# jujuC31/NeutFEM

Hardware: AMD Instinct MI355X
Metric: outer power-iters/sec (IAEA-3D RT0-P0 k-eigenvalue solve) (higher is better)
Workload: dtype f64; 1 GPU; IAEA-3D resampled 256x256x256 RT0-P0 2g, full Schur path, CG tol 0.0001, Chebyshev; cells=16777216, groups=2, parallelism=1 process(es) x 1 z-slab(s) each; RCCL: interface planes + scalar all-reduces

## Files before the change

### neutfem_amd/csrc/neutfem_hip.hip

```cpp
#include "../../include/neutfem_hip.h"
#include "nf_kernels.h"
#include "nf_assembly.h"
#include "nf_line_groups.h"
#include "nf_options.h"
#include "nf_small_eig.h"

#include <dlfcn.h>
#include <unistd.h>

#include <algorithm>
#include <chrono>
#include <climits>
#include <cmath>
#include <cstdarg>
#include <cstdint>
#include <cstdio>
#include <cstdlib>
#include <cstring>
#include <map>
#include <mutex>
#include <string>
#include <type_traits>
#include <utility>
#include <vector>

using namespace nf;

static thread_local std::string g_err;
static int fail(int code, const char *fmt, ...)
{
    char buf[512]; va_list ap; va_start(ap, fmt); vsnprintf(buf, sizeof buf, fmt, ap); va_end(ap);
    g_err = buf; return code;
}
#define HIPCHK(x) do { hipError_t e_ = (x); if (e_ != hipSuccess) return fail(NF_ERR_HIP, "%s failed: %s (%s:%d)", #x, hipGetErrorString(e_), __FILE__, __LINE__); } while (0)
#define NFCHK(x) do { int r_ = (x); if (r_ != NF_OK) return r_; } while (0)

static_assert(NF_OPT_RED_GRID == 1024, "nf_options.h: defaults and cap of the reduction-shaped grids follow RED_GRID");
static const int RED_GRID = 1024;
static const int MAX_LOCAL_SLABS = 16;

struct ProfSlot {
    std::vector<float> samples;
    void stats(long *count, double *ms, long *skipped) const
    {
        *count = 0; *ms = 0.0; *skipped = 0;
        if (samples.empty()) return;
        std::vector<float> v(samples); std::nth_element(v.begin(), v.begin() + v.size() / 2, v.end());
        const double thr = 0.25 * v[v.size() / 2];
        for (float x : samples) { if (x < thr) ++*skipped; else { ++*count; *ms += x; } }
    }
};

typedef struct ncclComm *ncclComm_t;
typedef struct { char internal[128]; } ncclUniqueId;
struct Rccl {
    void *lib = nullptr;
    int (*GetUniqueId)(ncclUniqueId *) = nullptr;
    int (*CommInitRank)(ncclComm_t *, int, ncclUniqueId, int) = nullptr;
// ... 2 lines not shown
    int (*Send)(const void *, size_t, int, int, ncclComm_t, hipStream_t) = nullptr;
    int (*Recv)(void *, size_t, int, int, ncclComm_t, hipStream_t) = nullptr;
    int (*GroupStart)() = nullptr;
    int (*GroupEnd)() = nullptr;
    const char *(*GetErrorString)(int) = nullptr;
    int (*CommAbort)(ncclComm_t) = nullptr;
    int (*CommCount)(const ncclComm_t, int *) = nullptr;
    char path[512] = { 0 };
};
static Rccl g_rccl;
static bool trace_comm() { static int on = -1; if (on < 0) { const char *e = getenv("NEUTFEM_TRACE_COMM"); on = e && atoi(e) ? 1 : 0; } return on == 1; }
#define TRACE_COMM(...) do { if (trace_comm()) { fprintf(stderr, "[comm] " __VA_ARGS__); fputc('\n', stderr); } } while (0)
static const int NCCL_DOUBLE = 8, NCCL_SUM = 0, NCCL_MAX = 2;
#define NCCLCHK(x) do { int r_ = (x); if (r_ != 0) return fail(NF_ERR_HIP, "%s failed: %s", #x, g_rccl.GetErrorString ? g_rccl.GetErrorString(r_) : "rccl error"); } while (0)

static int rccl_load()
{
    if (g_rccl.lib) return NF_OK;
    const char *env = getenv("NEUTFEM_RCCL_LIB");
    const char *names[] = { env ? env : "/opt/rocm/lib/librccl.so.1", "/opt/rocm/lib/librccl.so.1", "librccl.so.1", "librccl.so" };
    for (const char *n : names) { g_rccl.lib = dlopen(n, RTLD_NOW | RTLD_LOCAL); if (g_rccl.lib) break; }
    if (!g_rccl.lib) return fail(NF_ERR_HIP, "cannot load librccl.so: %s", dlerror());
#define SYM(field, name) do { *(void **)(&g_rccl.field) = dlsym(g_rccl.lib, name); if (!g_rccl.field) return fail(NF_ERR_HIP, "librccl.so lacks %s", name); } while (0)
    SYM(GetUniqueId, "ncclGetUniqueId"); SYM(CommInitRank, "ncclCommInitRank"); SYM(CommDestroy, "ncclCommDestroy");
    SYM(AllReduce, "ncclAllReduce"); SYM(Send, "ncclSend"); SYM(Recv, "ncclRecv"); SYM(GroupStart, "ncclGroupStart");
    SYM(GroupEnd, "ncclGroupEnd"); SYM(GetErrorString, "ncclGetErrorString");
#undef SYM
    *(void **)(&g_rccl.CommAbort) = dlsym(g_rccl.lib, "ncclCommAbort");
    *(void **)(&g_rccl.CommCount) = dlsym(g_rccl.lib, "ncclCommCount");
    Dl_info di;
    if (dladdr((void *)g_rccl.AllReduce, &di) && di.dli_fname) snprintf(g_rccl.path, sizeof g_rccl.path, "%s", di.dli_fname);
    return NF_OK;
}

struct nf_solver;
struct Transient;
struct nf_team {
    NfOptions opt;
    std::vector<nf_solver *> slabs;
    int device = 0;
    hipStream_t stream = nullptr;
    hipStream_t comm_stream = nullptr;
    hipStream_t y_stream = nullptr; hipEvent_t ev_fork = nullptr, ev_join = nullptr;
    hipEvent_t ev_z1 = nullptr, ev_xchg = nullptr;
    int nproc = 1, rank = 0;
    ncclComm_t comm = nullptr;
    ncclComm_t comm_x = nullptr;
    int last_cg_reductions = 0; long team_max_cells = 0;
    int last_cg_form = 0;
    int last_endpoint_w = 0;
    bool rccl_reduce = false;
    double *d_partials = nullptr; long partial_stride = 0, slab_cap = 0;
    CgScalars *d_cg = nullptr;
    double *d_out = nullptr;
    double *d_red = nullptr;
    double *d_errsrc = nullptr;
    double *d_vec = nullptr; long vec_stride = 0;
    int vec_cnt_pq = 0, vec_cnt_rr = 0; bool vec_ok = false; int last_vec_reduce = 0;
    bool dead = false;
    bool poisoned = false; int poison_rc = 0; char poison_msg[256] = { 0 };
    int xchg_in_apply = 0;
    long cg_iter_total = 0;
    int inject_rank = -1; long inject_iter = -1;
    int inject_outer = -1; char inject_where = 0;
    double comm_timeout_s = 120.0;
    nf_progress_fn progress_fn = nullptr; void *progress_user = nullptr;
    volatile long outers_done = 0;
    bool linked_ready = false;
    int sep_sweeps = 0;
    std::vector<int> last_its;
    int last_outer = 0, coarse_outer = 0; long last_cg_total = 0;
    std::vector<double> hist_k, hist_dk, hist_dphi; std::vector<int> hist_cg;
    int has_valid_keff = 0; double last_keff = 1.0;
    HostPub *h_pub = nullptr, *d_pub = nullptr; unsigned long long pub_seq = 0;
    bool profile = false; long prof_tick = 0;
    std::map<std::string, ProfSlot> prof;
    struct Ev { hipEvent_t a, b; int slot; };
    std::vector<Ev> ev_pending; std::vector<std::pair<hipEvent_t, hipEvent_t>> ev_free;
    OuterState *d_ost = nullptr; double *d_hist = nullptr; int hist_cap = 0;
    int ncu = 256;
    size_t lds_limit = 160 * 1024;
    int last_xcd = 0; long xcd_solves = 0, xcd_refused = 0;
    XcdState *d_xcd = nullptr; double *d_xpart = nullptr;
    int last_resident_serial = 0;
    int *d_hist_cg = nullptr; int hist_cg_cap = 0; ResidentOut *d_rout = nullptr;
    int last_path = 0;
    int last_direct = 0;
    long standin_unconverged = 0;
    std::vector<nf_solver *> cc; int cc_f[3] = {0, 0, 0};
};

struct nf_solver {
    int device = 0;
    nf_team *team = nullptr;
    int slab_index = 0;
    int if_lo = 0, if_hi = 0;
    int dim = 1, nx = 1, ny = 1, nz = 1, ng = 1, k = 0, m = 0;
    int n1 = 1, nloc = 1, nb = 0;
    long N = 0, nphi = 0, nJ = 0, nJx = 0, nJy = 0, nJz = 0;
    std::vector<double> xb, yb, zb, hx, hy, hz;
    double *d_hx = nullptr, *d_hy = nullptr, *d_hz = nullptr, *d_xb = nullptr, *d_yb = nullptr, *d_zb = nullptr;
    int bc_set[8] = {0}, bc_type[8] = {0};
    double *d_D = nullptr, *d_SigR = nullptr, *d_NSF = nullptr, *d_Chi = nullptr;
    std::vector<double *> d_SigS;
    bool xs_uploaded = false, built = false, diag_valid = false;
    unsigned char *d_void = nullptr; std::vector<unsigned char> void_host; double void_gamma = 0.0; long void_cells = 0;
    double *d_Cd = nullptr, *d_Mf = nullptr, *d_Mchi = nullptr;
    double *d_phi_adj = nullptr;
    double *d_modes[2] = {nullptr, nullptr}; int modes_n[2] = {0, 0}, modes_cap[2] = {0, 0};
    int has_valid_adjoint = 0; double last_keff_adj = 1.0;
    double *d_gamma = nullptr, *d_gpt_w = nullptr, *d_gpt_sc = nullptr; bool gpt_valid = false;
    std::vector<double *> d_Ms;
    const double **d_Ms_tab = nullptr;
    double *d_L[3] = {nullptr, nullptr, nullptr}, *d_DR[3] = {nullptr, nullptr, nullptr}, *d_D0[3] = {nullptr, nullptr, nullptr};
    long nlines[3] = {0, 0, 0};
    bool ld_tried = false, ld_use[3] = {false, false, false}; int ld_rejected = 0, ld_pitch[3] = {0, 0, 0};
    int *d_lid[3] = {nullptr, nullptr, nullptr}; double *d_ltab[3] = {nullptr, nullptr, nullptr};
    std::vector<long> ld_off[3]; std::vector<int> ld_rows[3]; size_t ld_bytes = 0;
    double *d_Sinv = nullptr;
    double *d_Sdense = nullptr; bool dense_valid = false;
    double *d_alo = nullptr, *d_ahi = nullptr, *d_hlo = nullptr, *d_hhi = nullptr, *d_gfl = nullptr;
    double *d_sinv_lo = nullptr, *d_sinv_hi = nullptr;
    double *d_clo = nullptr, *d_chi = nullptr, *d_rlo = nullptr, *d_rhi = nullptr, *d_ulo = nullptr, *d_uhi = nullptr;
    double *d_ctlo = nullptr, *d_cthi = nullptr, *d_elo = nullptr, *d_ehi = nullptr, *d_relo = nullptr, *d_rehi = nullptr;
    double *d_Wlo = nullptr, *d_Whi = nullptr; bool w_valid = false;
    double *d_phi = nullptr, *d_raw = nullptr;
    double *d_p0 = nullptr, *d_p1 = nullptr;
    double *d_tf = nullptr, *d_rhs = nullptr, *d_r = nullptr, *d_p = nullptr, *d_q = nullptr;
    double *d_p2 = nullptr, *d_qy = nullptr, *d_qz = nullptr;
    bool raw_valid = false, raw_is_diag = false;
    double *d_qsrc = nullptr;
    double src_total = 0.0; bool src_any = false;
    Transient *tr = nullptr; long build_gen = 0;
    long tr_rebuilds = 0;
    int opt_tr_rebalance = 1;
    double *d_Jz = nullptr; bool jz_valid = false;
    double *d_Jzb = nullptr;
    bool cmfd_init = false, cmfd_iface = false; double cmfd_relax = 1.0;
    double *d_Dt[3] = {nullptr, nullptr, nullptr}, *d_Dh[3] = {nullptr, nullptr, nullptr}; long nfc[3] = {0, 0, 0};
    double *d_cm = nullptr, *d_cmJ = nullptr; CmfdScalars *d_cmsc = nullptr;
    int cmfd_last_its = 0;
};

const char *nf_last_error(void) { return g_err.c_str(); }

static void coarse_cache_drop(nf_team *T)
{
    if (!T || T->cc.empty()) return;
    std::string keep = g_err;
    std::vector<nf_solver *> cc; cc.swap(T->cc);
    for (int i = (int)cc.size() - 1; i >= 0; --i) if (cc[i]) nf_destroy(cc[i]);
    g_err = keep;
}

int nf_device_count(void)
{
    int n = 0;
    if (hipGetDeviceCount(&n) != hipSuccess) { (void)hipGetLastError(); return 0; }
    return n;
}

template <class T> static int dalloc(T **p, size_t n)
{
    if (*p) { (void)hipFree(*p); *p = nullptr; }
    HIPCHK(hipMalloc((void **)p, std::max<size_t>(n, 1) * sizeof(T)));
    return NF_OK;
}
template <class T> static void dfree(T *&p) { if (p) { (void)hipFree(p); p = nullptr; } }
template <class T> struct DevTmp { T *p = nullptr; ~DevTmp() { if (p) (void)hipFree(p); } DevTmp() = default; DevTmp(const DevTmp &) = delete; DevTmp &operator=(const DevTmp &) = delete; };

static void line_dict_drop(nf_solver *S)
{
    if (S->team && S->team->stream && (S->d_lid[0] || S->d_lid[1] || S->d_lid[2])) (void)hipStreamSynchronize(S->team->stream);
    for (int d = 0; d < 3; ++d) { dfree(S->d_lid[d]); dfree(S->d_ltab[d]); S->ld_use[d] = false; S->ld_pitch[d] = 0; S->ld_off[d].clear(); S->ld_rows[d].clear(); }
    S->ld_tried = false; S->ld_rejected = 0; S->ld_bytes = 0;
}

static void modes_drop(nf_solver *S);
static void gpt_drop(nf_solver *S);
static void transient_drop(nf_solver *S);
static bool team_is_single(const nf_team *T);
// ... 37 lines not shown
    long g = (n + block - 1) / block; if (g < 1) g = 1; if (g > cap) g = cap; return (int)g;
}

static int n_modes(const nf_solver *S) { int n = 1; for (int t = 1; t < S->dim; ++t) n *= S->n1; return n; }
static int moment_index(const nf_solver *S, int d, int mode, int i, double *Ta)
{
    const int n1 = S->n1;
    int idx[3] = {0, 0, 0}; double ta = 1.0; int q = mode;
    for (int t = 0; t < S->dim; ++t) {
        if (t == d) { idx[t] = i; continue; }
        idx[t] = q % n1; q /= n1;
        ta *= 2.0 / (2.0 * idx[t] + 1.0);
    }
    if (Ta) *Ta = ta;
    return idx[0] + n1 * idx[1] + n1 * n1 * idx[2];
}
static ModeArgs mode_args(const nf_solver *S, int g, int d, int mode, const double *xb, double *yb)
{
    ModeArgs ma; memset(&ma, 0, sizeof ma);
    double Ta = 1.0;
    for (int i = 0; i <= S->nb; ++i) {
        const int p = moment_index(S, d, mode, i, &Ta);
        ma.x[i] = xb + (long)p * S->N; ma.y[i] = yb + (long)p * S->N; ma.Cd[i] = S->d_Cd + (long)g * S->nphi + (long)p * S->N;
    }
    ma.Ta = Ta; ma.dir = d; ma.D = S->d_D + (long)g * S->N;
    ma.eL[0] = 5.0 / 8.0; ma.eR[0] = 5.0 / 8.0; ma.Gc[0] = -4.0 / 3.0; ma.iM[0] = 15.0 / 16.0;
    ma.eL[1] = -7.0 / 8.0; ma.eR[1] = 7.0 / 8.0; ma.Gc[1] = -4.0 / 5.0; ma.iM[1] = 105.0 / 16.0;
    return ma;
}
static ModeTab mode_tab(const nf_solver *S, int d)
{
    ModeTab mt; memset(&mt, 0, sizeof mt);
    mt.n = n_modes(S);
    for (int m = 0; m < mt.n; ++m)
        for (int i = 0; i <= S->nb; ++i) {
            double Ta = 1.0;
            const int p = moment_index(S, d, m, i, &Ta), p0 = moment_index(S, d, 0, i, nullptr);
            mt.Ta[m] = Ta; mt.doff[m][i] = (long)(p - p0) * S->N;
        }
    return mt;
}

static long slab_partial_need(const nf_solver *S)
{
    return (std::max<long>(RED_GRID, S->nlines[0] + (long)((S->nx + 7) / 8) * ((long)S->ny + S->nz)) + 16) * n_modes(S);
}
static int team_alloc(nf_team *T)
{
    long cap = 0;
    for (auto *S : T->slabs) cap = std::max(cap, slab_partial_need(S));
    T->slab_cap = cap; T->partial_stride = cap * (long)T->slabs.size();
    NFCHK(dalloc(&T->d_partials, (size_t)T->partial_stride * 4));
    if (!T->d_cg) NFCHK(dalloc(&T->d_cg, 1));
    if (!T->d_out) NFCHK(dalloc(&T->d_out, 8));
    if (!T->d_red) NFCHK(dalloc(&T->d_red, 8));
    if (!T->d_errsrc) { NFCHK(dalloc(&T->d_errsrc, 1)); HIPCHK(hipMemset(T->d_errsrc, 0, sizeof(double))); }
    if (const char *e = getenv("NEUTFEM_INJECT_FAIL")) {
        int r = -1, ml = 0; long it = -1; char w = 0; int on = -1;
        if (sscanf(e, "%d:%c%d", &r, &w, &on) >= 2 && (w == 'o' || w == 'e' || w == 'a')) { T->inject_rank = r; T->inject_where = w; T->inject_outer = on; }
        else {
            const int nf = sscanf(e, "%d:%ld:%d", &r, &it, &ml);
            if (nf >= 2 && (nf < 3 || T->slabs.empty() || T->slabs[0]->nloc >= ml)) { T->inject_rank = r; T->inject_iter = it; }
        }
    }
    if (const char *e = getenv("NEUTFEM_COMM_TIMEOUT_S")) { const double v = atof(e); if (v > 0) T->comm_timeout_s = v; }
    T->last_its.assign(64, 0);
    return NF_OK;
}
static void team_free(nf_team *T)
{
    if (!T) return;
    (void)hipSetDevice(T->device);
    if (T->dead) {
        delete T;
        return;
    }
    if (T->stream) (void)hipStreamSynchronize(T->stream);
    for (auto &e : T->ev_pending) { (void)hipEventDestroy(e.a); (void)hipEventDestroy(e.b); }
    for (auto &e : T->ev_free) { (void)hipEventDestroy(e.first); (void)hipEventDestroy(e.second); }
    if (T->comm_x && g_rccl.CommDestroy) g_rccl.CommDestroy(T->comm_x);
    if (T->comm && g_rccl.CommDestroy) g_rccl.CommDestroy(T->comm);
    if (T->d_xcd) (void)hipFree(T->d_xcd);
    dfree(T->d_xpart);
    dfree(T->d_partials); dfree(T->d_cg); dfree(T->d_out); dfree(T->d_red); dfree(T->d_errsrc); dfree(T->d_vec); dfree(T->d_ost); dfree(T->d_hist); dfree(T->d_hist_cg); dfree(T->d_rout);
    if (T->h_pub) (void)hipHostFree(T->h_pub);
    if (T->comm_stream) { (void)hipStreamSynchronize(T->comm_stream); (void)hipStreamDestroy(T->comm_stream); }
    if (T->y_stream) { (void)hipStreamSynchronize(T->y_stream); (void)hipStreamDestroy(T->y_stream); }
    if (T->ev_fork) (void)hipEventDestroy(T->ev_fork);
    if (T->ev_join) (void)hipEventDestroy(T->ev_join);
    if (T->ev_z1) (void)hipEventDestroy(T->ev_z1);
    if (T->ev_xchg) (void)hipEventDestroy(T->ev_xchg);
    if (T->stream) (void)hipStreamDestroy(T->stream);
    delete T;
}
static PartSegs segs_for(const nf_team *T, const std::vector<int> &counts)
{
    PartSegs ps; ps.n = (int)T->slabs.size();
    for (int i = 0; i < ps.n; ++i) { ps.off[i] = (int)(i * T->slab_cap); ps.cnt[i] = counts[i]; }
    return ps;
}

static int create_impl(int rt_order, int p_order, int ng, int nxb, const double *xb, int nyb, const double *yb, int nzb,
                       const double *zb, int if_lo, int if_hi, int device, nf_handle *out)
{
    if (!out || !xb || nxb < 2 || ng < 1 || ng > 64) return fail(NF_ERR_ARG, "nf_create: bad arguments");
    int k = std::min(rt_order, 2), m = std::min(p_order, 2);
    if (k < m) m = k;
    int ndev = nf_device_count();
    if (ndev <= 0) return fail(NF_ERR_NO_DEVICE, "nf_create: no HIP device visible (the gfx950 path has no CPU fallback)");
    if (device < 0 || device >= ndev) return fail(NF_ERR_ARG, "nf_create: device %d out of range (%d devices)", device, ndev);
    HIPCHK(hipSetDevice(device));
    nf_solver *S = new nf_solver();
    S->device = device; S->k = k; S->m = m; S->ng = ng; S->if_lo = if_lo; S->if_hi = if_hi;
    S->xb.assign(xb, xb + nxb);
    if (nyb > 1) S->yb.assign(yb, yb + nyb); else S->yb.assign(1, nyb == 1 && yb ? yb[0] : 0.0);
    if (nzb > 1) S->zb.assign(zb, zb + nzb); else S->zb.assign(1, nzb == 1 && zb ? zb[0] : 0.0);
    S->nx = nxb - 1; S->ny = nyb > 1 ? nyb - 1 : 1; S->nz = nzb > 1 ? nzb - 1 : 1;
    S->dim = S->nz > 1 ? 3 : (S->ny > 1 ? 2 : 1);
    if ((if_lo || if_hi) && (S->dim != 3 || S->nz < 3)) { delete S; return fail(NF_ERR_ARG, "a slab needs a 3D mesh with at least 3 z-planes"); }
    if (S->dim == 3 && (nyb < 2 || !yb)) { delete S; return fail(NF_ERR_ARG, "nf_create: a 3D mesh needs at least 2 y breaks (got %d)", nyb); }
    S->N = (long)S->nx * S->ny * S->nz;
    S->n1 = m + 1; S->nloc = 1; for (int t = 0; t < S->dim; ++t) S->nloc *= S->n1;
    S->nphi = S->N * S->nloc; S->nb = std::min(k, m);
    S->hx.resize(S->nx); S->hy.assign(S->ny, 1.0); S->hz.assign(S->nz, 1.0);
    for (int i = 0; i < S->nx; ++i) S->hx[i] = xb[i + 1] - xb[i];
    if (S->dim >= 2) for (int i = 0; i < S->ny; ++i) S->hy[i] = yb[i + 1] - yb[i];
    if (S->dim == 3) for (int i = 0; i < S->nz; ++i) S->hz[i] = zb[i + 1] - zb[i];
    for (auto *h : { &S->hx, &S->hy, &S->hz })
        for (double v : *h)
            if (!(v > 0.0) || !std::isfinite(v)) { delete S; return fail(NF_ERR_ARG, "nf_create: mesh breaks must be finite and strictly increasing (cell width %g)", v); }
    {
        int nf = 1, ni = k; for (int t = 1; t < S->dim; ++t) { nf *= k + 1; ni *= k + 1; }
        S->nJx = (long)(S->nx + 1) * S->ny * S->nz * nf;
        S->nJy = S->dim >= 2 ? (long)S->nx * (S->ny + 1) * S->nz * nf : 0;
        S->nJz = S->dim == 3 ? (long)S->nx * S->ny * (S->nz + 1) * nf : 0;
        S->nJ = S->nJx + S->nJy + S->nJz + S->N * S->dim * ni;
    }
// ... 46 lines not shown
    if (rc == NF_OK) rc = dalloc(&S->d_q, S->nphi);
    if (rc == NF_OK && (if_lo || if_hi)) {
        const size_t nl = (size_t)S->nlines[2] * n_modes(S);
        double **arrs[] = { &S->d_clo, &S->d_chi, &S->d_rlo, &S->d_rhi, &S->d_ulo, &S->d_uhi, &S->d_ctlo, &S->d_cthi, &S->d_elo, &S->d_ehi, &S->d_relo, &S->d_rehi };
        for (auto a : arrs) if (rc == NF_OK) { rc = dalloc(a, nl); if (rc == NF_OK) (void)hipMemset(*a, 0, nl * sizeof(double)); }
    }
    if (rc == NF_OK) rc = team_alloc(T);
    if (rc != NF_OK) { nf_destroy(S); *out = nullptr; return rc; }
    S->d_SigS.assign((size_t)ng * ng, nullptr); S->d_Ms.assign((size_t)ng * ng, nullptr);
    return nf_reset_flux(S);
}

int nf_create(int rt_order, int p_order, int ng, int nxb, const double *xb, int nyb, const double *yb, int nzb,
              const double *zb, int device, nf_handle *out)
{
    return create_impl(rt_order, p_order, ng, nxb, xb, nyb, yb, nzb, zb, 0, 0, device, out);
}
int nf_create_slab(int rt_order, int p_order, int ng, int nxb, const double *xb, int nyb, const double *yb, int nzb,
                   const double *zb_slab, int interface_below, int interface_above, int device, nf_handle *out)
{
    return create_impl(rt_order, p_order, ng, nxb, xb, nyb, yb, nzb, zb_slab, interface_below ? 1 : 0, interface_above ? 1 : 0, device, out);
}

int nf_destroy(nf_handle S)
{
    if (!S) return NF_OK;
    (void)hipSetDevice(S->device);
    nf_team *T = S->team;
    if (T && T->dead) {
        std::vector<nf_solver *> cc; cc.swap(T->cc);
        for (auto *c : cc) if (c) nf_destroy(c);
        T->slabs.erase(std::remove(T->slabs.begin(), T->slabs.end(), S), T->slabs.end());
        if (T->slabs.empty()) team_free(T);
        delete S;
        return NF_OK;
    }
    coarse_cache_drop(T);
    transient_drop(S);
    if (T && T->stream) (void)hipStreamSynchronize(T->stream);
    for (int d = 0; d < 3; ++d) { dfree(S->d_Dt[d]); dfree(S->d_Dh[d]); }
    dfree(S->d_cm); dfree(S->d_cmJ); dfree(S->d_cmsc);
    dfree(S->d_hx); dfree(S->d_hy); dfree(S->d_hz); dfree(S->d_xb); dfree(S->d_yb); dfree(S->d_zb);
    dfree(S->d_D); dfree(S->d_SigR); dfree(S->d_NSF); dfree(S->d_Chi); dfree(S->d_void);
    for (auto &p : S->d_SigS) dfree(p);
    for (auto &p : S->d_Ms) dfree(p);
    dfree(S->d_Ms_tab);
    dfree(S->d_Cd); dfree(S->d_Mf); dfree(S->d_Mchi); dfree(S->d_phi_adj); dfree(S->d_Sinv); dfree(S->d_Sdense);
    for (int d = 0; d < 3; ++d) { dfree(S->d_L[d]); dfree(S->d_DR[d]); dfree(S->d_D0[d]); dfree(S->d_lid[d]); dfree(S->d_ltab[d]); }
    dfree(S->d_alo); dfree(S->d_ahi); dfree(S->d_hlo); dfree(S->d_hhi); dfree(S->d_gfl); dfree(S->d_sinv_lo); dfree(S->d_sinv_hi);
    dfree(S->d_clo); dfree(S->d_chi); dfree(S->d_rlo); dfree(S->d_rhi); dfree(S->d_ulo); dfree(S->d_uhi);
    dfree(S->d_Wlo); dfree(S->d_Whi);
    dfree(S->d_Jz); dfree(S->d_Jzb); dfree(S->d_ctlo); dfree(S->d_cthi); dfree(S->d_elo); dfree(S->d_ehi); dfree(S->d_relo); dfree(S->d_rehi);
    dfree(S->d_phi); dfree(S->d_raw); dfree(S->d_p0); dfree(S->d_p1);
    dfree(S->d_tf); dfree(S->d_rhs); dfree(S->d_r); dfree(S->d_p); dfree(S->d_q); dfree(S->d_p2); dfree(S->d_qy); dfree(S->d_qz);
    dfree(S->d_qsrc); dfree(S->d_modes[0]); dfree(S->d_modes[1]);
    dfree(S->d_gamma); dfree(S->d_gpt_w); dfree(S->d_gpt_sc);
    if (T) {
        T->slabs.erase(std::remove(T->slabs.begin(), T->slabs.end(), S), T->slabs.end());
        for (size_t i = 0; i < T->slabs.size(); ++i) T->slabs[i]->slab_index = (int)i;
        if (T->slabs.empty()) team_free(T);
    }
    delete S;
    return NF_OK;
}

int nf_link_slabs(nf_handle *handles, int n)
{
    if (!handles || n < 1 || n > MAX_LOCAL_SLABS) return fail(NF_ERR_ARG, "nf_link_slabs: 1..%d slabs", MAX_LOCAL_SLABS);
    nf_solver *S0 = handles[0];
    if (!S0) return fail(NF_ERR_ARG, "nf_link_slabs: null handle");
    HIPCHK(hipSetDevice(S0->device));
    for (int i = 0; i < n; ++i) {
        nf_solver *S = handles[i];
        if (!S || S->team->slabs.size() != 1) return fail(NF_ERR_STATE, "nf_link_slabs: handle %d is null or already linked", i);
        if (S->device != S0->device || S->nx != S0->nx || S->ny != S0->ny || S->ng != S0->ng)
            return fail(NF_ERR_ARG, "nf_link_slabs: slab %d does not match slab 0 (device, nx, ny, groups)", i);
        if (i > 0 && (!S->if_lo || !handles[i - 1]->if_hi)) return fail(NF_ERR_ARG, "nf_link_slabs: slabs %d/%d lack the shared interface flag", i - 1, i);
    }
    nf_team *T = S0->team;
    for (int i = 0; i < n; ++i) coarse_cache_drop(handles[i]->team);
    for (int i = 1; i < n; ++i) {
        nf_solver *S = handles[i];
        team_free(S->team);
        S->team = T; S->slab_index = i; T->slabs.push_back(S);
    }
    T->linked_ready = false;
    return team_alloc(T);
}

int nf_comm_unique_id(void *id128)
{
    if (!id128) return fail(NF_ERR_ARG, "nf_comm_unique_id: null buffer");
    NFCHK(rccl_load());
    ncclUniqueId id; NCCLCHK(g_rccl.GetUniqueId(&id));
    memcpy(id128, &id, sizeof id);
    return NF_OK;
}
int nf_comm_init(nf_handle S, const void *id128, int nranks, int rank)
{
    if (!S || !id128 || nranks < 1 || rank < 0 || rank >= nranks) return fail(NF_ERR_ARG, "nf_comm_init: bad arguments");
    nf_team *T = S->team;
    const bool force = getenv("NEUTFEM_FORCE_RCCL") != nullptr;
    if (nranks == 1 && !force) { T->nproc = 1; T->rank = 0; return NF_OK; }
    NFCHK(rccl_load());
    HIPCHK(hipSetDevice(T->device));
    ncclUniqueId id; memcpy(&id, id128, sizeof id);
    NCCLCHK(g_rccl.CommInitRank(&T->comm, nranks, id, rank));
// ... 311 lines not shown
}
static void prof_collect(nf_team *T)
{
    for (auto &e : T->ev_pending) {
        float ms = 0.f;
        if (hipEventSynchronize(e.b) == hipSuccess && hipEventElapsedTime(&ms, e.a, e.b) == hipSuccess) T->prof[SLOT_NAMES[e.slot]].samples.push_back(ms);
        T->ev_free.push_back({e.a, e.b});
    }
    T->ev_pending.clear();
}

static int exchange_planes(nf_team *T, int which, int g, hipStream_t st)
{
    const int ns = (int)T->slabs.size();
    ++T->xchg_in_apply;
    auto send_lo = [&](nf_solver *S) { return which == 0 ? S->d_clo : which == 2 ? S->d_elo : S->d_hlo + (size_t)g * S->nlines[2]; };
    auto send_hi = [&](nf_solver *S) { return which == 0 ? S->d_chi : which == 2 ? S->d_ehi : S->d_hhi + (size_t)g * S->nlines[2]; };
    auto recv_lo = [&](nf_solver *S) { return which == 2 ? S->d_relo : S->d_rlo; };
    auto recv_hi = [&](nf_solver *S) { return which == 2 ? S->d_rehi : S->d_rhi; };
    for (int i = 0; i + 1 < ns; ++i) {
        nf_solver *A = T->slabs[i], *B = T->slabs[i + 1];
        const size_t bytes = (size_t)A->nlines[2] * (which == 1 ? 1 : n_modes(A)) * sizeof(double);
        HIPCHK(hipMemcpyAsync(recv_lo(B), send_hi(A), bytes, hipMemcpyDeviceToDevice, st));
        HIPCHK(hipMemcpyAsync(recv_hi(A), send_lo(B), bytes, hipMemcpyDeviceToDevice, st));
    }
    nf_solver *bot = T->slabs.front(), *top = T->slabs.back();
    if (T->nproc > 1 && (bot->if_lo || top->if_hi)) {
        const size_t cnt = (size_t)bot->nlines[2] * (which == 1 ? 1 : n_modes(bot));
        TRACE_COMM("rank %d exchange which=%d count=%zu lo=%d hi=%d poisoned=%d", T->rank, which, cnt, bot->if_lo, top->if_hi, (int)T->poisoned);
        ncclComm_t cx = T->comm_x ? T->comm_x : T->comm;
        NCCLCHK(g_rccl.GroupStart());
        if (bot->if_lo) {
            NCCLCHK(g_rccl.Send(send_lo(bot), cnt, NCCL_DOUBLE, T->rank - 1, cx, st));
            NCCLCHK(g_rccl.Recv(recv_lo(bot), cnt, NCCL_DOUBLE, T->rank - 1, cx, st));
        }
        if (top->if_hi) {
            NCCLCHK(g_rccl.Send(send_hi(top), cnt, NCCL_DOUBLE, T->rank + 1, cx, st));
            NCCLCHK(g_rccl.Recv(recv_hi(top), cnt, NCCL_DOUBLE, T->rank + 1, cx, st));
        }
        NCCLCHK(g_rccl.GroupEnd());
    } else if (bot->if_lo || top->if_hi) {
        return fail(NF_ERR_STATE, "slab %s has an interface but no neighbour: link the slabs (nf_link_slabs) or init the communicator (nf_comm_init)",
                    bot->if_lo ? "bottom" : "top");
    }
    return NF_OK;
}

struct ApplyCg {
    const CgScalars *cg = nullptr;
    bool fused = false; const std::vector<double *> *xsol = nullptr;
    CgLean lean = {};
    CgLean lean_z1 = {};
    Cg1 cg1 = {};
};
struct PassCg {
    const CgScalars *cg = nullptr; CgFuse fuse = {}; CgLean lean = {}, lean_z1 = {}; Cg1 cg1 = {};
    bool zw_dot = false;
    hipStream_t stream = nullptr;
    bool noacc = false; const double *yadd = nullptr;
};
static PassCg pass_cg(const ApplyCg &A, const nf_solver *S, int i) { return { A.cg, A.fused ? CgFuse{ S->d_p, S->d_r, (*A.xsol)[i] } : CgFuse{}, A.lean, A.lean_z1, A.cg1 }; }
struct SegPlan { int rc = NF_OK, SEG = 0, NSEG = 0, TX = 0, nparts = 0; dim3 grid, block; size_t lds = 0; };
static SegPlan seg_plan(const nf_solver *S, int d, int zmode);
static int launch_s(const nf_solver *S, int d, int g, const ModeArgs &ma, const Geom &G, int last, double *partials, const PassCg &P, int *nparts, int zmode);
static int line_dict_prepare(nf_team *T);
static int team_prepare(nf_team *T)
{
    NFCHK(line_dict_prepare(T));
    if (T->linked_ready) return NF_OK;
    if (T->opt.xchg_comm && T->nproc > 1 && T->comm && !T->comm_x) {
        ncclUniqueId id2; memset(&id2, 0, sizeof id2);
        double v[128]; for (double &x : v) x = 0.0;
        if (T->rank == 0) { NCCLCHK(g_rccl.GetUniqueId(&id2)); for (int i = 0; i < 128; ++i) v[i] = (double)(unsigned char)id2.internal[i]; }
        DevTmp<double> d; NFCHK(dalloc(&d.p, 128));
        HIPCHK(hipMemcpyAsync(d.p, v, sizeof v, hipMemcpyHostToDevice, T->stream));
        NCCLCHK(g_rccl.AllReduce(d.p, d.p, 128, NCCL_DOUBLE, NCCL_SUM, T->comm, T->stream));
        HIPCHK(hipMemcpyAsync(v, d.p, sizeof v, hipMemcpyDeviceToHost, T->stream));
        NFCHK(team_stream_wait(T, T->stream));
        for (int i = 0; i < 128; ++i) id2.internal[i] = (char)(unsigned char)v[i];
        NCCLCHK(g_rccl.CommInitRank(&T->comm_x, T->nproc, id2, T->rank));
        TRACE_COMM("rank %d: second communicator for the plane exchange", T->rank);
    }
    bool any = false;
    for (auto *S : T->slabs) { if (!S->built) return fail(NF_ERR_STATE, "every slab must be built (nf_build) before solving"); any |= S->if_lo || S->if_hi; }
    if (any) {
        const int ng = T->slabs[0]->ng;
        for (int g = 0; g < ng; ++g) {
            NFCHK(exchange_planes(T, 1, g, T->stream));
            for (auto *S : T->slabs) {
                const long nl = S->nlines[2];
                const unsigned gr = (unsigned)((nl + 255) / 256);
                if (S->if_lo) hipLaunchKernelGGL(k_sred_inv, dim3(gr), dim3(256), 0, T->stream, S->d_hlo + g * nl, S->d_rlo, S->d_sinv_lo + g * nl, nl, 0);
                if (S->if_hi) hipLaunchKernelGGL(k_sred_inv, dim3(gr), dim3(256), 0, T->stream, S->d_hhi + g * nl, S->d_rhi, S->d_sinv_hi + g * nl, nl, 1);
            }
            NFCHK(team_stream_wait(T, T->stream));
        }
        double worst = 0.0; int worst_nz = 0;
        for (auto *S : T->slabs) {
            if (!(S->if_lo && S->if_hi)) continue;
            const size_t nl = (size_t)S->nlines[2] * ng;
            std::vector<double> gfl(nl), slo(nl), shi(nl);
            HIPCHK(hipMemcpy(gfl.data(), S->d_gfl, nl * sizeof(double), hipMemcpyDeviceToHost));
            HIPCHK(hipMemcpy(slo.data(), S->d_sinv_lo, nl * sizeof(double), hipMemcpyDeviceToHost));
            HIPCHK(hipMemcpy(shi.data(), S->d_sinv_hi, nl * sizeof(double), hipMemcpyDeviceToHost));
            for (size_t i = 0; i < nl; ++i) {
                const double w = std::fabs(gfl[i]) * std::sqrt(std::fabs(slo[i] * shi[i]));
                if (w > worst) { worst = w; worst_nz = S->nz; }
            }
        }
        if (T->rccl_reduce && T->nproc > 1) {
            HIPCHK(hipMemcpyAsync(T->d_red, &worst, sizeof(double), hipMemcpyHostToDevice, T->stream));
            NCCLCHK(g_rccl.AllReduce(T->d_red, T->d_red, 1, NCCL_DOUBLE, NCCL_MAX, T->comm, T->stream));
            HIPCHK(hipMemcpyAsync(&worst, T->d_red, sizeof(double), hipMemcpyDeviceToHost, T->stream));
            NFCHK(team_stream_wait(T, T->stream));
// ... 13 lines not shown
    T->vec_ok = false;
    T->team_max_cells = 0; for (auto *X : T->slabs) T->team_max_cells = std::max(T->team_max_cells, X->N);
    if (T->rccl_reduce && T->nproc > 1) {
        nf_solver *S = T->slabs[0];
        const bool eligible = T->slabs.size() == 1 && S->nloc == 1 && S->dim == 3 && (S->if_lo || S->if_hi);
        int np = 0;
        if (eligible) {
            const SegPlan sp = seg_plan(S, 2, 2);
            np = sp.rc == NF_OK ? sp.nparts : 0;
        }
        const int nr = eligible ? grid_for(S->nphi) : 0;
        double v[5] = { (double)np, -(double)np, (double)nr, -(double)nr, (double)T->team_max_cells };
        HIPCHK(hipMemcpyAsync(T->d_red, v, sizeof v, hipMemcpyHostToDevice, T->stream));
        NCCLCHK(g_rccl.AllReduce(T->d_red, T->d_red, 5, NCCL_DOUBLE, NCCL_MAX, T->comm, T->stream));
        HIPCHK(hipMemcpyAsync(v, T->d_red, sizeof v, hipMemcpyDeviceToHost, T->stream));
        NFCHK(team_stream_wait(T, T->stream));
        T->team_max_cells = (long)v[4];
        T->vec_cnt_pq = np; T->vec_cnt_rr = nr;
        T->vec_stride = T->slab_cap + 2;
        T->vec_ok = eligible && v[0] == -v[1] && v[2] == -v[3] && np > 0 && np < T->slab_cap && nr > 0 && nr < T->slab_cap;
        if (T->vec_ok && !T->d_vec) { NFCHK(dalloc(&T->d_vec, (size_t)T->vec_stride * 2)); HIPCHK(hipMemset(T->d_vec, 0, (size_t)T->vec_stride * 2 * sizeof(double))); }
    }
    for (auto *S : T->slabs) S->w_valid = false;
    if (T->opt.endpoint_weights && T->opt.cg_single_reduce != 0 && (T->opt.cg_single_reduce > 0 || T->team_max_cells <= T->opt.cg_single_reduce_max_cells))
        for (auto *S : T->slabs) {
            if (!(S->if_lo || S->if_hi) || S->nb != 0 || S->dim != 3 || S->nloc != 1) continue;
            const size_t NG = (size_t)S->N * S->ng; const long nxy = S->nlines[2];
            if (!S->d_Wlo) { NFCHK(dalloc(&S->d_Wlo, NG)); NFCHK(dalloc(&S->d_Whi, NG)); }
            HIPCHK(hipMemsetAsync(S->d_Wlo, 0, NG * sizeof(double), T->stream)); HIPCHK(hipMemsetAsync(S->d_Whi, 0, NG * sizeof(double), T->stream));
            HIPCHK(hipMemsetAsync(S->d_p, 0, (size_t)S->N * sizeof(double), T->stream));
            const Geom G = make_geom(S);
            const unsigned gf = (unsigned)grid_for(nxy);
            for (int g = 0; g < S->ng; ++g)
                for (int k = 0; k < S->nz; ++k) {
                    double *plane = S->d_p + (size_t)k * nxy;
                    hipLaunchKernelGGL(k_fill_const, dim3(gf), dim3(256), 0, T->stream, plane, nxy, 1.0);
                    NFCHK(launch_s(S, 2, g, mode_args(S, g, 2, 0, S->d_p, S->d_q), G, 0, nullptr, PassCg(), nullptr, 1));
                    if (S->if_lo) HIPCHK(hipMemcpyAsync(S->d_Wlo + (size_t)g * S->N + (size_t)k * nxy, S->d_clo, (size_t)nxy * sizeof(double), hipMemcpyDeviceToDevice, T->stream));
                    if (S->if_hi) HIPCHK(hipMemcpyAsync(S->d_Whi + (size_t)g * S->N + (size_t)k * nxy, S->d_chi, (size_t)nxy * sizeof(double), hipMemcpyDeviceToDevice, T->stream));
                    hipLaunchKernelGGL(k_fill_const, dim3(gf), dim3(256), 0, T->stream, plane, nxy, 0.0);
                }
            HIPCHK(hipStreamSynchronize(T->stream));
            HIPCHK(hipGetLastError());
            S->w_valid = true;
        }
    T->linked_ready = true;
    return NF_OK;
}

static int team_finalize(nf_team *T, int op, const std::vector<int> &counts, int nq, double *out, double tol, int maxit, bool want_flag = false)
{
    PartSegs ps = segs_for(T, counts);
    if (!T->rccl_reduce) {
        hipLaunchKernelGGL(k_finalize, dim3(1), dim3(256), 0, T->stream, op, T->d_partials, ps, T->partial_stride, nq, T->d_cg, out, tol, maxit, 0, T->d_red, (const double *)nullptr);
    } else {
        hipLaunchKernelGGL(k_finalize, dim3(1), dim3(256), 0, T->stream, op, T->d_partials, ps, T->partial_stride, nq, T->d_cg, out, tol, maxit, 1, T->d_red, (const double *)T->d_errsrc);
        TRACE_COMM("rank %d allreduce finalize op=%d count=%d poisoned=%d", T->rank, op, nq + 1, (int)T->poisoned);
        NCCLCHK(g_rccl.AllReduce(T->d_red, T->d_red, (size_t)nq + 1, NCCL_DOUBLE, NCCL_SUM, T->comm, T->stream));
        hipLaunchKernelGGL(k_cg_logic, dim3(1), dim3(1), 0, T->stream, op, T->d_red, nq, T->d_cg, out, tol, maxit, want_flag ? 2 : 1);
    }
    return NF_OK;
}

static bool team_poison(nf_team *T, int code, bool vec_slots = false)
{
    if (code == NF_OK) return false;
    if (T->nproc <= 1) return true;
    if (!T->poisoned) {
        T->poisoned = true; T->poison_rc = code; snprintf(T->poison_msg, sizeof T->poison_msg, "%s", nf_last_error());
        const double one = 1.0;
        (void)hipMemcpyAsync(T->d_errsrc, &one, sizeof one, hipMemcpyHostToDevice, T->stream);
        if (vec_slots) for (double *slot : { T->d_partials + T->vec_cnt_pq, T->d_partials + T->partial_stride + T->vec_cnt_rr }) (void)hipMemcpyAsync(slot, &one, sizeof one, hipMemcpyHostToDevice, T->stream);
        (void)hipStreamSynchronize(T->stream);
        (void)hipGetLastError();
    }
    return false;
}
static int team_poison_result(nf_team *T)
{
    const int code = T->poison_rc; char msg[256]; snprintf(msg, sizeof msg, "%s", T->poison_msg);
    T->poisoned = false;
    (void)hipMemsetAsync(T->d_errsrc, 0, sizeof(double), T->stream);
    return fail(code, "%s", msg);
}
static int team_verdict(nf_team *T, int local_rc, const char *what)
{
    if (T->nproc > 1 && T->rank == T->inject_rank && T->inject_where == 'a') { T->inject_where = 0; local_rc = fail(NF_ERR_HIP, "injected failure on rank %d before %s (NEUTFEM_INJECT_FAIL)", T->rank, what); }
    if (!(T->rccl_reduce && T->nproc > 1)) return local_rc;
    std::string keep = local_rc != NF_OK ? g_err : std::string();
    double v = local_rc != NF_OK ? 1.0 : 0.0;
    HIPCHK(hipMemcpyAsync(T->d_red, &v, sizeof v, hipMemcpyHostToDevice, T->stream));
    TRACE_COMM("rank %d allreduce verdict before %s", T->rank, what);
    NCCLCHK(g_rccl.AllReduce(T->d_red, T->d_red, 1, NCCL_DOUBLE, NCCL_MAX, T->comm, T->stream));
    HIPCHK(hipMemcpyAsync(&v, T->d_red, sizeof v, hipMemcpyDeviceToHost, T->stream));
    NFCHK(team_stream_wait(T, T->stream));
    if (local_rc != NF_OK) { g_err = keep; return local_rc; }
    if (v != 0.0) return fail(NF_ERR_REMOTE, "another rank of the team reported an error before %s; no rank started it", what);
    return NF_OK;
}

static int team_reduce(nf_team *T, const std::vector<int> &counts, double *red)
{
    PartSegs ps = segs_for(T, counts);
    hipLaunchKernelGGL(k_finalize, dim3(1), dim3(256), 0, T->stream, (int)FIN_SUM, T->d_partials, ps, T->partial_stride, 1, T->d_cg, red, 0.0, 0, 1, red, (const double *)T->d_errsrc);
    if (T->rccl_reduce) { TRACE_COMM("rank %d allreduce reduce count=2 poisoned=%d", T->rank, (int)T->poisoned); NCCLCHK(g_rccl.AllReduce(red, red, 2, NCCL_DOUBLE, NCCL_SUM, T->comm, T->stream)); }
    return NF_OK;
}

static int team_reduce_sr(nf_team *T, const std::vector<int> &counts, const std::vector<int> &cnt3)
{
    PartSegs ps = segs_for(T, counts);
    std::vector<int> c3(counts);
    for (size_t i = 0; i < c3.size(); ++i) if (cnt3[i] > 0 && counts[i] > 0) c3[i] = cnt3[i];
    PartSegs ps3 = segs_for(T, c3);
    hipLaunchKernelGGL(k_reduce_rows, dim3(1), dim3(256), 0, T->stream, (const double *)T->d_partials, ps, ps3, T->partial_stride, T->d_red, (const double *)T->d_errsrc);
    if (T->rccl_reduce) { TRACE_COMM("rank %d allreduce single-reduction count=5 poisoned=%d", T->rank, (int)T->poisoned); NCCLCHK(g_rccl.AllReduce(T->d_red, T->d_red, 5, NCCL_DOUBLE, NCCL_SUM, T->comm, T->stream)); }
    return NF_OK;
}

static bool lds_opt_in(const void *fn, size_t lds)
{
    if (lds <= 64 * 1024) return true;
    static std::map<std::pair<int, const void *>, size_t> granted;
    static std::mutex mu;
    int dev = 0; (void)hipGetDevice(&dev);
    std::lock_guard<std::mutex> lock(mu);
    auto it = granted.find({ dev, fn });
    if (it != granted.end() && it->second >= lds) return true;
    if (hipFuncSetAttribute(fn, hipFuncAttributeMaxDynamicSharedMemorySize, (int)lds) != hipSuccess) { (void)hipGetLastError(); return false; }
    granted[{ dev, fn }] = lds;
    return true;
}
static bool nt_regime(const nf_solver *S) { return S->team->opt.nt_loads && S->N > S->team->opt.nt_min_cells; }
static bool x_nt(const nf_solver *S, int NB) { return NB == 0 && S->nx % 2 == 0 && nt_regime(S); }
static bool dict_dir(const nf_solver *S, int d) { return S->ld_use[d]; }
static const int X_DICT_MAX_NCH = 16;
static bool x_dict(const nf_solver *S, int NB, int NCH, bool nt) { return nt && NB == 0 && NCH <= X_DICT_MAX_NCH && dict_dir(S, 0); }
struct DictArgs { bool on = false; const double *L = nullptr, *DR = nullptr, *C = nullptr; LineDict ld; };
static DictArgs dict_args(const nf_solver *S, int d, int g, bool on)
{
    DictArgs A; A.on = on;
    if (!on) return A;
    const long rows = (long)S->ld_rows[d][g] * S->ld_pitch[d];
    A.L = S->d_ltab[d] + S->ld_off[d][g]; A.DR = A.L + rows; A.C = d == 0 ? A.DR + rows : nullptr;
    A.ld.id = S->d_lid[d] + (long)g * S->nlines[d]; A.ld.pitch = S->ld_pitch[d];
    return A;
}
static bool x_xcd(const nf_solver *S, bool nt) { return nt && S->team->opt.xcd >= 0 && (S->team->opt.xcd & 4); }
static bool x_fuses(const nf_solver *S) { return !(S->if_lo || S->if_hi); }
template <class F, unsigned I> static bool call_index(F &f) { return f(std::integral_constant<unsigned, I>()); }
template <class F, unsigned... I> static bool with_index(unsigned key, F &f, std::integer_sequence<unsigned, I...>)
{
    static constexpr bool (*tab[])(F &) = { &call_index<F, I>... };
    return key < sizeof...(I) && tab[key](f);
}
template <unsigned N, class F> static bool with_index(unsigned key, F &&f) { return with_index(key, f, std::make_integer_sequence<unsigned, N>()); }

constexpr bool schur_x_legal(int NCH, bool VEC, int NB, bool NT, bool DICT)
{
    return NCH >= 1 && NCH <= (NB == 0 ? 32 : 8) && (NCH & (NCH - 1)) == 0 && NB >= 0 && NB <= 2
        && (!NT || (VEC && NB == 0)) && (!DICT || (NT && NCH <= X_DICT_MAX_NCH));
}
struct XPlan { int lpl_log2 = 0, NCH = 0; unsigned grid = 0; bool vec = false, nt = false, xcd = false, dict = false; };
static XPlan x_plan(const nf_solver *S)
{
    XPlan P; const int K = 2;
    const int lanes = (S->nx + K - 1) / K;
    while ((1 << P.lpl_log2) < lanes && P.lpl_log2 < 6) ++P.lpl_log2;
    const int LPL = 1 << P.lpl_log2, LPW = 64 / LPL;
    const int nch = (S->nx + LPL * K - 1) / (LPL * K);
    P.grid = (unsigned)((S->nlines[0] + 4 * LPW - 1) / (4 * LPW));
    for (int c = 1; c <= (S->nb == 0 ? 32 : 8); c *= 2) if (nch <= c) { P.NCH = c; break; }
    P.vec = S->nx % 2 == 0; P.nt = x_nt(S, S->nb);
    P.xcd = x_xcd(S, P.nt); P.dict = x_dict(S, S->nb, P.NCH, P.nt);
    return P;
}
static int launch_x(const nf_solver *S, int g, const ModeArgs &ma0, const Geom &G, int last, double *partials, const PassCg &P, int *nparts)
{
    const XPlan xp = x_plan(S);
    if (!xp.NCH) return fail(NF_ERR_UNSUPPORTED, "nx = %d exceeds the x-line kernel limit (%d cells)", S->nx, S->nb == 0 ? 4096 : 1024);
    if (nparts) *nparts = (int)xp.grid * n_modes(S);
    const CgFuse fz = x_fuses(S) ? P.fuse : CgFuse{ nullptr, nullptr, nullptr };
    const ModeTab mt = mode_tab(S, 0);
    const dim3 gr(xp.grid, (unsigned)mt.n);
    const int first = 1 | (xp.xcd ? 2 : 0);
    const DictArgs da = dict_args(S, 0, g, xp.dict);
    ModeArgs ma = ma0; if (da.on) ma.Cd[0] = da.C;
    const double *L = da.on ? da.L : S->d_L[0] + g * S->N, *DR = da.on ? da.DR : S->d_DR[0] + g * S->N, *D0 = S->d_D0[0] + g * S->nlines[0];
    int lg = 0; while ((1 << lg) < xp.NCH) ++lg;
    const unsigned key = ((((unsigned)lg * 3 + (unsigned)S->nb) * 2 + xp.vec) * 2 + xp.nt) * 2 + xp.dict;
    const bool hit = with_index<6 * 3 * 8>(key, [&](auto i) {
        constexpr unsigned I = decltype(i)::value;
        constexpr int NCH = 1 << (I / 24), NB = I / 8 % 3; constexpr bool VEC = I & 4, NT = I & 2, DICT = I & 1;
        if constexpr (!schur_x_legal(NCH, VEC, NB, NT, DICT)) return false;
        else hipLaunchKernelGGL((k_schur_x<2, NCH, VEC, NB, NT, DICT>), gr, dim3(256), 0, S->team->stream, ma, mt, G, L, DR, D0, S->nx, S->ny, S->nlines[0], xp.lpl_log2,
                                first, last, partials, P.cg, fz, P.lean, da.ld);
        return true;
    });
    return hit ? NF_OK : fail(NF_ERR_ARG, "k_schur_x: no instantiation for NCH = %d, NB = %d, vec %d, nt %d, dict %d", xp.NCH, S->nb, xp.vec, xp.nt, xp.dict);
}

struct ChunkPlan { bool ok = false; int NS = 0, TX = 0; size_t lds = 0; };
static ChunkPlan chunk_plan(const nf_solver *S, int d)
{
    ChunkPlan P; const nf_team *T = S->team;
    const int n = d == 1 ? S->ny : S->nz;
    if (S->nb != 0 || d < 1 || d >= S->dim || (d == 2 && (S->if_lo || S->if_hi)) || !((T->opt.s_long_dirs >> (d - 1)) & 1)) return P;
    const int nmin = d == 1 ? T->opt.s_long_min_y : T->opt.s_long_min;
    if (!(T->opt.s_long == 1 || (T->opt.s_long < 0 && n > nmin)) || (size_t)S->N * sizeof(double) >= (1ull << 32)) return P;
    P.NS = (n + 15) / 16;
    P.TX = T->opt.s_tx ? T->opt.s_tx : 32;
    while (P.TX > 8 && P.TX * P.NS > 1024) P.TX >>= 1;
    while (P.TX > 8 && P.TX / 2 >= S->nx) P.TX >>= 1;
    P.lds = (size_t)(3 * P.TX * P.NS + 2 * P.TX + 16 + 2 * 8 * P.NS * P.TX) * sizeof(double);
    P.ok = P.TX * P.NS <= 1024 && P.lds <= T->lds_limit;
    if (P.ok && n <= 256 && T->opt.s_long < 1) {
        const long tiles = (long)((S->nx + P.TX - 1) / P.TX) * (d == 1 ? S->nz : S->ny);
        if (tiles < 1024) P.ok = false;
    }
    return P;
}

static dim3 c_grid(const nf_solver *S, int d, const ChunkPlan &cp) { return dim3((unsigned)((S->nx + cp.TX - 1) / cp.TX), (unsigned)(d == 1 ? S->nz : S->ny)); }
static unsigned c_block(const ChunkPlan &cp) { return (unsigned)((cp.TX * cp.NS + 63) / 64 * 64); }
static const int C_SEG = 8, C_NCH = 2;
static bool c_nt(const nf_solver *S) { return nt_regime(S); }
static bool c_dict(const nf_solver *S, int d, bool nt) { return nt && dict_dir(S, d); }
static const int C_EARLY_AUTO = 2;
static int c_early(const nf_solver *S, bool dict) { const int e = S->team->opt.c_early; return dict ? (e < 0 ? C_EARLY_AUTO : e) : 0; }
static int c_xcd(const nf_solver *S, int d, bool nt) { const nf_team *T = S->team; return T->opt.xcd >= 0 ? (T->opt.xcd >> (d - 1)) & 1 : (d == 1 && nt); }
static int s_xcd(const nf_solver *S, int d, int zmode)
{
    const nf_team *T = S->team;
    return T->opt.xcd >= 0 ? (T->opt.xcd >> (d - 1)) & 1 : ((d == 1 && nt_regime(S)) || ((zmode == 1 || zmode == 2) && S->N <= (6L << 20)));
}
static bool s_nt(const nf_solver *S, int zmode, int SEG) { return zmode != 3 && S->nb == 0 && SEG == 8 && nt_regime(S); }
static bool s_dict(const nf_solver *S, int d, int zmode, int SEG) { return zmode == 0 && s_nt(S, zmode, SEG) && dict_dir(S, d); }
static bool s_zw(const nf_solver *S, int zmode, bool zw_dot, bool want_dot) { return zmode == 0 && S->nb == 0 && zw_dot && want_dot; }
static const int S_STAGE_AUTO_DIRS = 2;
static size_t s_stage_bytes(int n, int TX) { const int rpp = 1024 / (8 * TX); return (size_t)((n + rpp - 1) / rpp) * 1024; }
static unsigned s_stage_blocks(const nf_solver *S, const SegPlan &sp)
{
    const unsigned tiles = sp.grid.x * sp.grid.y, want = (unsigned)(S->team->opt.s_stage_grid > 0 ? S->team->opt.s_stage_grid : S->team->ncu);
    return std::min(tiles, want);
}
static bool s_stage(const nf_solver *S, int d, int zmode, const SegPlan &sp, unsigned V)
{
    const nf_team *T = S->team;
    if (zmode != 0 || T->opt.s_stage == 0 || !(V & SV_NT) || !(V & SV_DICT) || (V & ~(SV_NT | SV_DICT | SV_ZW))) return false;
    if (sp.TX < 8 || sp.TX > 64 || (sp.TX & (sp.TX - 1)) || S->nx % sp.TX != 0) return false;
    if (sp.lds + s_stage_bytes(d == 1 ? S->ny : S->nz, sp.TX) > T->lds_limit) return false;
    if (T->opt.s_stage > 0) return true;
// ... 270 lines not shown
            hipLaunchKernelGGL(k_sep_couple, gr, dim3(256), 0, T->comm_stream, S->d_gfl + g * nl, S->d_ulo, S->d_uhi, S->d_elo, S->d_ehi, nl, nl * n_modes(S), S->if_lo, S->if_hi, cg); });
        NFCHK(exchange_planes(T, 2, 0, T->comm_stream));
        each_slab([&](nf_solver *S, long nl, dim3 gr) {
            hipLaunchKernelGGL(k_sep_update, gr, dim3(256), 0, T->comm_stream, S->d_ctlo, S->d_cthi, S->d_elo, S->d_ehi, S->d_relo, S->d_rehi,
                               S->d_sinv_lo + g * nl, S->d_sinv_hi + g * nl, S->d_ulo, S->d_uhi, nl, nl * n_modes(S), S->if_lo, S->if_hi, cg); });
    }
    HIPCHK(hipEventRecord(T->ev_xchg, T->comm_stream));
    return NF_OK;
}

static bool team_is_single(const nf_team *T) { return T->slabs.size() == 1 && !T->slabs[0]->if_lo && !T->slabs[0]->if_hi; }
static bool split_dot(const nf_team *T, bool want_dot, bool lean)
{
    const int dim = T->slabs[0]->dim;
    bool split = want_dot && dim >= 2 && team_is_single(T) && T->slabs[0]->nb == 0 && !lean && T->opt.split_dot;
    if (split && T->opt.split_dot < 2) split = chunk_plan(T->slabs[0], dim - 1).ok;
    return split;
}
static bool xy_overlap(const nf_team *T, bool any_if, bool prof)
{
    const bool xy = T->slabs[0]->dim == 3 && any_if && T->opt.xy_overlap && T->slabs[0]->nb == 0 && T->y_stream && !prof;
    bool xy_all = xy; if (xy) for (auto *X : T->slabs) xy_all = xy_all && X->N <= T->opt.xy_overlap_max_cells && !chunk_plan(X, 1).ok;
    return xy_all;
}

static int team_schur_apply(nf_team *T, int g, const std::vector<const double *> &xs, const std::vector<double *> &ys, bool want_dot,
                            const ApplyCg &A, std::vector<int> *counts = nullptr, std::vector<int> *cnt3 = nullptr)
{
    const int ns = (int)T->slabs.size();
    const int dim = T->slabs[0]->dim;
    bool any_if = false; for (auto *S : T->slabs) any_if |= S->if_lo || S->if_hi;
    hipEvent_t a, b, ta = nullptr, tb = nullptr;
    const bool prof = T->profile && (T->prof_tick++ % T->opt.prof_every == 0);
    if (prof) prof_begin(T, 3, &ta, &tb);
    if (any_if) {
        if (prof) prof_begin(T, 4, &a, &b);
        NFCHK(team_endpoint_phase(T, g, xs, ys, A, prof ? b : nullptr, false, cnt3));
    }
    const bool split = split_dot(T, want_dot, A.lean.st != nullptr);
    std::vector<int> totals(ns, 0);
    for (int d = 0; d < dim; ++d) {
        const int last = d == dim - 1;
        if (d == 2 && any_if) HIPCHK(hipStreamWaitEvent(T->stream, T->ev_xchg, 0));
        if (prof) prof_begin(T, d, &a, &b);
        const bool xy_all = xy_overlap(T, any_if, prof);
        if (d == 0 && xy_all) { HIPCHK(hipEventRecord(T->ev_fork, T->stream)); HIPCHK(hipStreamWaitEvent(T->y_stream, T->ev_fork, 0)); }
        if (d == 2 && xy_all) { HIPCHK(hipEventRecord(T->ev_join, T->y_stream)); HIPCHK(hipStreamWaitEvent(T->stream, T->ev_join, 0)); }
        for (int i = 0; i < ns; ++i) {
            nf_solver *S = T->slabs[i];
            const Geom G = make_geom(S);
            if (xy_all && !S->d_qy) NFCHK(dalloc(&S->d_qy, S->nphi));
            {
                double *part = (want_dot && (last || split)) ? T->d_partials + i * T->slab_cap + totals[i] : nullptr;
                const ModeArgs ma = mode_args(S, g, d, 0, xs[i], ys[i]);
                int np = 0;
                PassCg P = pass_cg(A, S, i); P.zw_dot = split;
                if (d == 0) NFCHK(launch_x(S, g, ma, G, last || split, part, P, &np));
                else if (d == 2 && (S->if_lo || S->if_hi)) {
                    P.yadd = xy_all ? S->d_qy : nullptr;
                    NFCHK(launch_s(S, 2, g, ma, G, last, part, P, &np, 2));
                } else if (d == 1 && xy_all) {
                    P.stream = T->y_stream; P.noacc = true;
                    NFCHK(launch_s(S, 1, g, mode_args(S, g, 1, 0, xs[i], S->d_qy), G, 0, nullptr, P, &np, 0));
                } else NFCHK(launch_s(S, d, g, ma, G, last || split, part, P, &np, 0));
                if (part) totals[i] += np;
            }
            if (counts && last) (*counts)[i] = totals[i];
        }
        if (prof) (void)hipEventRecord(b, T->stream);
    }
    if (prof) (void)hipEventRecord(tb, T->stream);
    return NF_OK;
}


int nf_schur_apply(nf_handle S, int g, const double *x_dev, double *y_dev)
{
    if (!S || !x_dev || !y_dev || g < 0 || g >= S->ng) return fail(NF_ERR_ARG, "nf_schur_apply: bad arguments");
    if (!S->built) return fail(NF_ERR_STATE, "nf_schur_apply: call nf_build first");
    nf_team *T = S->team;
    if (!team_is_single(T)) return fail(NF_ERR_STATE, "nf_schur_apply works on an undivided mesh; use nf_team_schur_apply for slabs");
    HIPCHK(hipSetDevice(S->device));
    NFCHK(line_dict_prepare(T));
    NFCHK(team_schur_apply(T, g, { x_dev }, { y_dev }, false, ApplyCg()));
    if (S->d_void) hipLaunchKernelGGL(k_void_apply_fix, dim3(grid_for(S->nphi)), dim3(256), 0, T->stream, x_dev, y_dev, (const double *)(S->d_Cd + (size_t)g * S->nphi), S->nphi, VoidMask{ S->d_void, S->N });
    HIPCHK(hipGetLastError());
    HIPCHK(hipStreamSynchronize(T->stream));
    if (T->profile) prof_collect(T);
    return NF_OK;
}

int nf_team_schur_apply(nf_handle S, int g, const double *const *x_dev, double *const *y_dev)
{
    if (!S || !x_dev || !y_dev || g < 0 || g >= S->ng) return fail(NF_ERR_ARG, "nf_team_schur_apply: bad arguments");
    if (S->team->dead) return fail(NF_ERR_COMM, "this team lost a collective (NF_ERR_COMM) and is unusable: destroy the handles and end the process with a non-zero code (never re-exec)");
    nf_team *T = S->team;
    HIPCHK(hipSetDevice(T->device));
    NFCHK(team_prepare(T));
    std::vector<const double *> xs(x_dev, x_dev + T->slabs.size()); std::vector<double *> ys(y_dev, y_dev + T->slabs.size());
    NFCHK(team_schur_apply(T, g, xs, ys, false, ApplyCg()));
    HIPCHK(hipGetLastError());
    HIPCHK(hipStreamSynchronize(T->stream));
    if (T->profile) prof_collect(T);
    return NF_OK;
}

#ifdef NF_STAMPS
static long long *g_stamps = nullptr;
extern "C" int nf_debug_stamps(long long *out48) { if (!g_stamps) return -1; return hipMemcpy(out48, g_stamps, 48 * sizeof(long long), hipMemcpyDeviceToHost) == hipSuccess ? 0 : -2; }
#endif
struct Fuse3Plan { bool ok = false; int nch = 1, vec = 1, seg = 8, B = 256, nblocks = 0; size_t lds = 0; Apply3 A; };
static Fuse3Plan fuse3_plan(const nf_solver *S)
{
    Fuse3Plan P; memset(&P.A, 0, sizeof P.A);
    const int K = 2, modes = n_modes(S);
    int lanes = (S->nx + K - 1) / K, lpl_log2 = 0;
// ... 90 lines not shown
    while ((1 << lpl_log2) < lanes && lpl_log2 < 5) ++lpl_log2;
    int nch = (lanes + (1 << lpl_log2) - 1) >> lpl_log2;
    if (nch == 1 && lpl_log2 == 5) {
        const int Pn = T->opt.cg_xcd_groups, tasks = (int)((S->nlines[0] + 1) / 2) * A.nmodes;
        int waves = (tasks + Pn - 1) / Pn;
        for (int r = 0; r < 2; ++r) if (S->dim >= r + 2) waves += (((P.A.gx[r] * P.A.gy[r] * A.nmodes + Pn - 1) / Pn) * P.A.TX[r] * P.A.NSEG[r] + 63) / 64;
        if (waves > XCD_THREADS / 64) { lpl_log2 = 4; nch = 2; }
    }
    if (nch > 2) return fail(NF_ERR_STATE, "k_cg_xcd: x lines of %d cells", S->nx);
    A.lpl_log2 = lpl_log2; A.ntask_x = (int)((S->nlines[0] + (64 >> lpl_log2) - 1) / (64 >> lpl_log2));
    for (int r = 0; r < 2; ++r) { A.n[r] = P.A.n[r]; A.TX[r] = P.A.TX[r]; A.NSEG[r] = P.A.NSEG[r]; A.gx[r] = P.A.gx[r]; A.gy[r] = P.A.gy[r]; A.sl[r] = P.A.sl[r]; A.ostride[r] = P.A.ostride[r]; }
    if (S->dim < 2) { A.TX[0] = A.NSEG[0] = 1; } if (S->dim < 3) { A.TX[1] = A.NSEG[1] = 1; }
    A.pA = S->d_p; A.pB = S->d_p2; A.r = S->d_r;
    A.part = T->d_xpart; A.st = T->d_xcd; A.xcc = T->opt.cg_xcd_id;
    *nch_out = nch;
    return NF_OK;
}
constexpr bool xcd_legal(int NCH, int NB, int SEG) { return NCH >= 1 && NCH <= 2 && NB >= 0 && NB <= 2 && SEG == (NB == 0 ? 8 : 4); }
template <int NCH_, bool VEC_, int NB_, int SEG_> struct XcdInst { static constexpr int NCH = NCH_, NB = NB_, SEG = SEG_; static constexpr bool VEC = VEC_; };
template <class F> static int xcd_select(const char *name, const nf_solver *S, const Fuse3Plan &P, int nch, F &&launch)
{
    int rc = NF_OK;
    const unsigned key = (P.seg == 4 || P.seg == 8) ? ((((unsigned)(nch - 1) * 2 + (P.vec ? 1u : 0u)) * 3 + (unsigned)S->nb) * 2 + (P.seg == 8 ? 1u : 0u)) : ~0u;
    const bool hit = with_index<2 * 2 * 3 * 2>(key, [&](auto i) {
        constexpr unsigned I = decltype(i)::value;
        constexpr int NCH = 1 + I / 12, NB = I / 2 % 3, SEG = (I & 1) ? 8 : 4; constexpr bool VEC = I / 6 % 2;
        if constexpr (!xcd_legal(NCH, NB, SEG)) return false;
        else { rc = launch(XcdInst<NCH, VEC, NB, SEG>()); return true; }
    });
    return hit ? rc : fail(NF_ERR_ARG, "%s: no instantiation for NCH = %d, vec %d, NB = %d, SEG = %d", name, nch, P.vec, S->nb, P.seg);
}
static const size_t XCD_LDS = (size_t)(5 * 1024 + 64 + 32) * sizeof(double);
static int launch_cg_xcd(nf_solver *S, int g, const Fuse3Plan &P, double *xsol, unsigned long long seq)
{
    nf_team *T = S->team; hipStream_t st = T->stream;
    XcdArgs A; int nch = 1;
    NFCHK(xcd_fill(S, g, P, A, &nch));
    A.xsol = xsol; A.cg = T->d_cg; A.hp = T->d_pub; A.seq = seq;
    const size_t lds = XCD_LDS; const unsigned G = 8u * (unsigned)T->opt.cg_xcd_groups;
    NFCHK(xcd_select("k_cg_xcd", S, P, nch, [&](auto t) -> int { using I = decltype(t);
        if (!lds_opt_in((const void *)k_cg_xcd<I::NCH, I::VEC, I::NB, I::SEG>, lds)) return fail(NF_ERR_HIP, "k_cg_xcd: %zu bytes of LDS refused", lds);
        hipLaunchKernelGGL((k_cg_xcd<I::NCH, I::VEC, I::NB, I::SEG>), dim3(G), dim3(XCD_THREADS), lds, st, A);
        return NF_OK;
    }));
    HIPCHK(hipGetLastError());
    return NF_OK;
}
enum CgForm { CG_XCD, CG_FUSE3, CG_LEAN, CG_FUSED, CG_CLASSIC, CG_TEAM_LEAN, CG_TEAM_VEC, CG_TEAM_SR };
static const char *const CG_FORM_NAME[] = { "xcd", "fuse3", "lean", "fused", "classic", "team_lean", "team_vec", "team_sr" };
struct CgPlan {
    CgForm form = CG_CLASSIC; Fuse3Plan f3; int gru = 0;
    bool fused = false; int reductions = 0;
    bool lean() const { return form == CG_XCD || form == CG_FUSE3 || form == CG_LEAN; }
};
static CgPlan cg_plan(const nf_team *T)
{
    CgPlan P; const nf_solver *S0 = T->slabs[0]; const bool single = team_is_single(T);
    P.fused = T->opt.cg_fuse != 0 && (single || S0->nloc == 1);
    P.reductions = single ? 0 : 2;
    P.form = P.fused ? CG_FUSED : CG_CLASSIC;
    if (!P.fused || !T->opt.cg_lean) return P;
    if (!single) {
        bool sr = T->opt.cg_single_reduce > 0 || (T->opt.cg_single_reduce < 0 && T->team_max_cells <= T->opt.cg_single_reduce_max_cells);
        for (auto *S : T->slabs) sr = sr && S->dim == 3 && S->nb == 0 && (T->opt.s_seg == 0 || T->opt.s_seg == 8) && S->nz <= 1024;
        const bool vec = T->nproc > 1 && T->slabs.size() == 1 && T->vec_ok && T->opt.vec_reduce;
        P.form = sr ? CG_TEAM_SR : vec ? CG_TEAM_VEC : CG_TEAM_LEAN; P.reductions = sr ? 1 : 2;
        return P;
    }
    if (T->rccl_reduce || S0->N > T->opt.cg_lean_max_cells) return P;
    P.form = CG_LEAN;
    P.gru = grid_for(S0->nphi, 256, T->opt.cg_lean_grid);
    if (!T->opt.cg_fuse3 || S0->N > T->opt.cg_fuse3_max_cells) return P;
    P.f3 = fuse3_plan(S0);
    if (P.f3.ok && P.f3.nblocks > T->slab_cap) P.f3.ok = false;
    if (P.f3.ok) P.form = xcd_eligible(T, S0, P.f3) ? CG_XCD : CG_FUSE3;
    return P;
}

struct PlanPass { const char *dir, *family; int mode, SEG, NCH, TX, NSEG; dim3 grid; unsigned block; bool nt, zw, order; unsigned tiles; bool fold = false, dict = false; int early = 0; unsigned V = 0, blocks = 0; int full = 0; };
static void plan_emit(std::string &js, const PlanPass &p)
{
    char tmp[416];
    snprintf(tmp, sizeof tmp, "%s{\"dir\": \"%s\", \"mode\": %d, \"family\": \"%s\", \"SEG\": %d, \"NCH\": %d, \"TX\": %d, \"NSEG\": %d, \"grid\": [%u, %u, %u], "
             "\"block\": %u, \"nt\": %d, \"zw\": %d, \"xcd_order\": %d, \"xcd_permutes\": %d, \"fold\": %d, \"dict\": %d, \"early\": %d", js.back() == '[' ? "" : ", ", p.dir, p.mode, p.family,
             p.SEG, p.NCH, p.TX, p.NSEG, p.grid.x, p.grid.y, p.grid.z, p.block, p.nt ? 1 : 0, p.zw ? 1 : 0, p.order ? 1 : 0, xcd_permutes(p.order, p.tiles) ? 1 : 0, p.fold ? 1 : 0, p.dict ? 1 : 0, p.early);
    js += tmp;
    if (!strcmp(p.family, "s")) js += ", \"variant\": \"" + variant_name(p.V) + "\"";
    if (p.dir[0] != 'x') js += ", \"stage\": " + std::to_string((p.V & SV_STAGE) && !strcmp(p.family, "s") ? 1 : 0) + ", \"blocks\": " + std::to_string(p.blocks)
                            + ", \"full\": " + std::to_string(p.full);
    js += "}";
}
static int plan_s(std::string &js, const nf_solver *S, int d, int zmode, bool want_dot, bool zw_dot, bool fuse, bool cg1)
{
    const SPass ps = s_pass(S, d, zmode, want_dot, zw_dot, fuse, cg1);
    if (ps.rc != NF_OK) return ps.rc;
    const dim3 gr = ps.chunked ? c_grid(S, d, ps.cp) : ps.seg.grid;
    plan_emit(js, { d == 1 ? "y" : "z", ps.chunked ? "c" : "s", zmode, ps.chunked ? C_SEG : ps.seg.SEG, ps.chunked ? C_NCH : 1, ps.chunked ? ps.cp.TX : ps.seg.TX, ps.chunked ? ps.cp.NS : ps.seg.NSEG,
                    gr, ps.chunked ? c_block(ps.cp) : ps.seg.block.x, (ps.V & SV_NT) != 0, (ps.V & SV_ZW) != 0, ps.xcd != 0, gr.x * gr.y, ps.fold, (ps.V & SV_DICT) != 0, ps.early, ps.V,
                    !ps.chunked && (ps.V & SV_STAGE) ? s_stage_blocks(S, ps.seg) * gr.z : gr.x * gr.y * gr.z, ps.full });
    return NF_OK;
}
int nf_apply_plan(nf_handle S, int in_cg, char *json_buf, size_t len)
{
    if (!S || !json_buf || len < 2) return fail(NF_ERR_ARG, "nf_apply_plan: bad arguments");
    if (!S->built) return fail(NF_ERR_STATE, "nf_apply_plan: call nf_build first");
    HIPCHK(hipSetDevice(S->team->device));
    NFCHK(line_dict_prepare(S->team));
    const nf_team *T = S->team;
    const bool slab = S->if_lo || S->if_hi;
    if (!team_is_single(T) && !T->linked_ready) return fail(NF_ERR_STATE, "nf_apply_plan: run a team apply or solve first (the team has not been prepared since its options changed)");
    const CgPlan cp = cg_plan(T);
    const bool cg = in_cg != 0, fused = cg && cp.fused, lean = cg && cp.lean(), sr = cg && cp.form == CG_TEAM_SR;
    const bool split = split_dot(T, cg, lean);
    bool any_if = false; for (auto *X : T->slabs) any_if |= X->if_lo || X->if_hi;
    const bool xy_all = xy_overlap(T, any_if, false);
    char tmp[288];
    snprintf(tmp, sizeof tmp, "{\"in_cg\": %d, \"form\": \"%s\", \"slab\": %d, \"fused\": %d, \"lean\": %d, \"single_reduce\": %d, \"split_dot\": %d, \"xy_overlap\": %d, \"passes\": [",
             cg ? 1 : 0, cg ? CG_FORM_NAME[cp.form] : "", slab ? 1 : 0, fused ? 1 : 0, lean ? 1 : 0, sr ? 1 : 0, split ? 1 : 0, xy_all ? 1 : 0);
    std::string js = tmp;
    for (int d = 0; d < S->dim; ++d) {
        const bool last = d == S->dim - 1, want_dot = cg && (last || split);
        if (d == 0) {
            const XPlan xp = x_plan(S);
            if (!xp.NCH) return fail(NF_ERR_UNSUPPORTED, "nx = %d exceeds the x-line kernel limit (%d cells)", S->nx, S->nb == 0 ? 4096 : 1024);
            plan_emit(js, { "x", "x", 0, 0, xp.NCH, 1 << xp.lpl_log2, 0, dim3(xp.grid, (unsigned)n_modes(S)), 256u, xp.nt, false, xp.xcd, xp.grid, false, xp.dict });
        } else if (d == 2 && slab) {
            if (endpoint_w_taken(T, S, sr, fused)) { const dim3 gr = endpoint_w_grid(S); plan_emit(js, { "z", "endpoint_w", 1, 0, 0, 64, 0, gr, 256u, false, false, false, gr.x * gr.y }); }
            else NFCHK(plan_s(js, S, 2, 1, false, false, fused, sr));
            NFCHK(plan_s(js, S, 2, 2, want_dot, split, fused, sr));
        } else if (d == 1 && xy_all) NFCHK(plan_s(js, S, 1, 0, false, split, fused, sr));
        else NFCHK(plan_s(js, S, d, 0, want_dot, split, fused, sr));
    }
    {
        int nd[3] = { 0, 0, 0 };
        for (int d = 0; d < S->dim; ++d) if (dict_dir(S, d)) nd[d] = *std::max_element(S->ld_rows[d].begin(), S->ld_rows[d].end());
        snprintf(tmp, sizeof tmp, "], \"line_dict\": {\"x\": %d, \"y\": %d, \"z\": %d}}", nd[0], nd[1], nd[2]);
        js += tmp;
    }
    if (js.size() + 1 > len) return fail(NF_ERR_ARG, "nf_apply_plan: buffer of %zu bytes is too small (%zu needed)", len, js.size() + 1);
    memcpy(json_buf, js.c_str(), js.size() + 1);
    return NF_OK;
}

struct CgRun {
    nf_team *T; int g; const CgPlan &P; CgForm form; const std::vector<double *> &x;
    std::vector<const double *> ps; std::vector<double *> qs;
    std::vector<int> gcnt, acnt, cnt3;
    bool any_if = false;
    double *row1() const { return T->d_partials + T->partial_stride; }
    double *vec_rr() const { return T->d_vec + T->vec_stride; }
    int chk(int rc) const { return team_poison(T, rc, form == CG_TEAM_VEC) ? rc : NF_OK; }
    template <class F> void each_slab(F &&launch) const { if (!T->poisoned) for (size_t i = 0; i < T->slabs.size(); ++i) launch(T->slabs[i], (int)i); }
};
static ApplyCg cg_apply_args(const CgRun &R, int index)
{
    nf_team *T = R.T; const int first = index == 0 ? 1 : 0;
    ApplyCg A; A.cg = T->d_cg; A.fused = R.P.fused; A.xsol = &R.x;
    if (R.form == CG_FUSE3 || R.form == CG_LEAN) A.lean = CgLean{ T->d_cg, R.row1(), R.P.gru, index & 1, first };
    if (R.form == CG_TEAM_SR) A.cg1 = Cg1{ T->d_red, T->d_cg, index };
    if (R.form == CG_TEAM_VEC) A.lean_z1 = CgLean{ T->d_cg, R.vec_rr(), T->vec_cnt_rr, index & 1, first, T->vec_cnt_rr };
    if (R.form == CG_TEAM_LEAN) A.lean_z1 = CgLean{ T->d_cg, T->d_red + 2, -1, index & 1, first };
    return A;
}
static int cg_step_fuse3(CgRun &R, int index)
{
    nf_team *T = R.T; nf_solver *S0 = T->slabs[0];
    double *A = S0->d_p, *B = S0->d_p2;
    double *pin = (index == 0 || (index & 1)) ? A : B, *pout = pin == A ? B : A;
    hipEvent_t ta = nullptr, tb = nullptr;
    const bool prof = T->profile && (T->prof_tick++ % T->opt.prof_every == 0);
    if (prof) prof_begin(T, 3, &ta, &tb);
    const int rc = launch_apply3(S0, R.g, R.P.f3, pin, pout, R.x[0], cg_apply_args(R, index).lean);
    if (prof) (void)hipEventRecord(tb, T->stream);
    with_void(S0, [&](auto M, VoidMask vm) {
        hipLaunchKernelGGL(k_cg_rupdate3<decltype(M)::value>, dim3(R.P.gru), dim3(256), 0, T->stream, S0->d_r, (const double *)S0->d_q, (const double *)(S0->dim >= 2 ? S0->d_qy : nullptr),
                           (const double *)(S0->dim == 3 ? S0->d_qz : nullptr), S0->nphi, T->d_cg, R.row1(), CgLean{ T->d_cg, T->d_partials, R.P.f3.nblocks, index & 1, 0 }, vm); });
    return rc;
}
static int cg_step_apply(CgRun &R, int index, long global_it)
{
    nf_team *T = R.T;
    T->xchg_in_apply = 0;
    int ra = NF_OK;
    if (T->nproc > 1 && T->rank == T->inject_rank && global_it == T->inject_iter)
        { ra = fail(NF_ERR_HIP, "injected failure on rank %d at CG iteration %ld (NEUTFEM_INJECT_FAIL)", T->rank, global_it); TRACE_COMM("rank %d INJECT at %ld", T->rank, global_it); }
    else if (!T->poisoned) ra = team_schur_apply(T, R.g, R.ps, R.qs, true, cg_apply_args(R, index), &R.acnt, &R.cnt3);
    NFCHK(R.chk(ra));
    if (T->poisoned && R.any_if) {
        if (T->xchg_in_apply == 0) { (void)hipEventRecord(T->ev_z1, T->stream); (void)hipStreamWaitEvent(T->comm_stream, T->ev_z1, 0); }
        for (int k = T->xchg_in_apply; k < 1 + T->sep_sweeps; ++k) (void)exchange_planes(T, k == 0 ? 0 : 2, 0, T->comm_stream);
        (void)hipEventRecord(T->ev_xchg, T->comm_stream); (void)hipStreamWaitEvent(T->stream, T->ev_xchg, 0);
        for (size_t i = 0; i < R.acnt.size(); ++i) R.acnt[i] = R.cnt3[i] = 0;
    }
    return NF_OK;
}
static int cg_step_team_sr(CgRun &R, int) { return R.chk(team_reduce_sr(R.T, R.acnt, R.cnt3)); }
static int cg_step_team_vec(CgRun &R, int index)
{
    nf_team *T = R.T; double *send_pq = T->d_partials, *send_rr = R.row1(), *vec_pq = T->d_vec;
    auto allred = [&](double *send, double *recv, int cnt) -> int { NCCLCHK(g_rccl.AllReduce(send, recv, (size_t)cnt + 1, NCCL_DOUBLE, NCCL_SUM, T->comm, T->stream)); return NF_OK; };
    if (!T->poisoned && R.acnt[0] != T->vec_cnt_pq) NFCHK(R.chk(fail(NF_ERR_STATE, "vector reduce: the accumulation pass left %d partials, %d were agreed", R.acnt[0], T->vec_cnt_pq)));
    NFCHK(R.chk(allred(send_pq, vec_pq, T->vec_cnt_pq)));
    R.each_slab([&](nf_solver *S, int i) { hipLaunchKernelGGL(k_cg_rupdate<false>, dim3(R.gcnt[i]), dim3(256), 0, T->stream, S->d_r, S->d_q, S->nphi, T->d_cg, send_rr, CgLean{ T->d_cg, vec_pq, T->vec_cnt_pq, index & 1, 0, T->vec_cnt_pq }, VoidMask{ nullptr, 0 }); });
    return R.chk(allred(send_rr, R.vec_rr(), T->vec_cnt_rr));
}
static int cg_step_team_lean(CgRun &R, int index)
{
    nf_team *T = R.T;
    NFCHK(R.chk(team_reduce(T, R.acnt, T->d_red)));
    R.each_slab([&](nf_solver *S, int i) { hipLaunchKernelGGL(k_cg_rupdate<false>, dim3(R.gcnt[i]), dim3(256), 0, T->stream, S->d_r, S->d_q, S->nphi, T->d_cg, T->d_partials + i * T->slab_cap, CgLean{ T->d_cg, T->d_red, -1, index & 1, 0 }, VoidMask{ nullptr, 0 }); });
    return R.chk(team_reduce(T, R.gcnt, T->d_red + 2));
}
static int cg_step_lean(CgRun &R, int index)
{
    R.each_slab([&](nf_solver *S, int) { with_void(S, [&](auto M, VoidMask vm) {
        hipLaunchKernelGGL(k_cg_rupdate<decltype(M)::value>, dim3(R.P.gru), dim3(256), 0, R.T->stream, S->d_r, S->d_q, S->nphi, R.T->d_cg, R.row1(), CgLean{ R.T->d_cg, R.T->d_partials, R.acnt[0], index & 1, 0 }, vm); }); });
    return NF_OK;
}
static int cg_step_scalar(CgRun &R, int)
{
    nf_team *T = R.T; const bool fused = R.form == CG_FUSED;
    NFCHK(R.chk(team_finalize(T, FIN_PAP, R.acnt, 1, T->d_out, 0.0, 0)));
    R.each_slab([&](nf_solver *S, int i) { with_void(S, [&](auto M, VoidMask vm) {
        if (fused) hipLaunchKernelGGL(k_cg_rupdate<decltype(M)::value>, dim3(R.gcnt[i]), dim3(256), 0, T->stream, S->d_r, S->d_q, S->nphi, T->d_cg, T->d_partials + i * T->slab_cap, CgLean{}, vm);
        else hipLaunchKernelGGL(k_cg_update<decltype(M)::value>, dim3(R.gcnt[i]), dim3(256), 0, T->stream, R.x[i], S->d_r, S->d_p, S->d_q, S->nphi, T->d_cg, T->d_partials + i * T->slab_cap, vm); }); });
    NFCHK(R.chk(team_finalize(T, FIN_RR, R.gcnt, 1, T->d_out, 0.0, 0)));
    if (!fused) R.each_slab([&](nf_solver *S, int i) { hipLaunchKernelGGL(k_cg_pupdate, dim3(R.gcnt[i]), dim3(256), 0, T->stream, S->d_p, S->d_r, S->nphi, T->d_cg); });
    return NF_OK;
}
static int cg_step(CgRun &R, int index, long global_it)
{
    static int (*const after_apply[])(CgRun &, int) = { nullptr, nullptr, cg_step_lean, cg_step_scalar, cg_step_scalar, cg_step_team_lean, cg_step_team_vec, cg_step_team_sr };
    if (R.form == CG_FUSE3) return cg_step_fuse3(R, index);
    NFCHK(cg_step_apply(R, index, global_it));
    return after_apply[R.form](R, index);
}
static int cg_stop_test(CgRun &R, int launched, CgScalars *sc)
{
    nf_team *T = R.T; const ApplyCg A = cg_apply_args(R, launched);
    if ((R.form == CG_FUSE3 || R.form == CG_LEAN) && pub_ready(T)) {
        const unsigned long long seq = ++T->pub_seq;
        hipLaunchKernelGGL(k_cg_lean_rr, dim3(1), dim3(256), 0, T->stream, A.lean, T->d_pub, seq);
        return pub_wait(T, seq, sc, nullptr, 0);
    }
    if (R.form == CG_FUSE3 || R.form == CG_LEAN) hipLaunchKernelGGL(k_cg_lean_rr, dim3(1), dim3(256), 0, T->stream, A.lean, (HostPub *)nullptr, 0ULL);
    if (R.form == CG_TEAM_SR) hipLaunchKernelGGL(k_cg1_logic, dim3(1), dim3(64), 0, T->stream, A.cg1, (HostPub *)nullptr, 0ULL);
    if (R.form == CG_TEAM_VEC || R.form == CG_TEAM_LEAN) hipLaunchKernelGGL(k_cg_lean_rr, dim3(1), dim3(256), 0, T->stream, A.lean_z1, (HostPub *)nullptr, 0ULL);
    return readback(T, T->d_cg, sc, nullptr, nullptr, 0);
}
static int cg_result(nf_team *T, int g, CgForm form, const CgScalars &sc, int *its_out, double *res_out)
{
    T->last_cg_form = form;
    if (!std::isfinite(sc.rr)) return fail(NF_ERR_NUMERIC, "CG produced a non-finite residual (group %d)", g);
    T->last_its[g] = sc.its;
    if (its_out) *its_out = sc.its;
    if (res_out) *res_out = sc.rhs_norm > 0 ? std::sqrt(sc.rr) / sc.rhs_norm : 0.0;
    return NF_OK;
}
static int cg_solve(nf_team *T, int g, const std::vector<const double *> &rhs, const std::vector<double *> &x, double tol, int maxit,
                    int *its_out, double *res_out, bool inited = false)
{
    const int ns = (int)T->slabs.size(); nf_solver *S0 = T->slabs[0];
    const CgPlan P = cg_plan(T);
    CgRun R{ T, g, P, P.form, x };
    R.ps.resize(ns); R.qs.resize(ns); R.gcnt.resize(ns); R.acnt.resize(ns); R.cnt3.assign(ns, 0);
    auto init = [&] { for (int i = 0; i < ns; ++i) with_void(T->slabs[i], [&](auto M, VoidMask vm) {
        hipLaunchKernelGGL(k_cg_init<decltype(M)::value>, dim3(R.gcnt[i]), dim3(256), 0, T->stream, rhs[i], x[i], T->slabs[i]->d_r, T->slabs[i]->d_p, T->slabs[i]->nphi, T->d_partials + i * T->slab_cap, vm); }); };
    for (int i = 0; i < ns; ++i) { nf_solver *S = T->slabs[i]; R.gcnt[i] = grid_for(S->nphi); R.ps[i] = S->d_p; R.qs[i] = S->d_q; R.any_if |= S->if_lo || S->if_hi; }
    if (!inited) init();
    NFCHK(team_finalize(T, FIN_RHS, R.gcnt, 1, T->d_out, tol, maxit));
    CgScalars sc; memset(&sc, 0, sizeof sc);
    T->last_cg_reductions = P.reductions; T->last_endpoint_w = 0; T->last_vec_reduce = P.form == CG_TEAM_VEC ? 1 : 0; T->last_xcd = 0;
    if (P.f3.ok) {
        if (!S0->d_p2) NFCHK(dalloc(&S0->d_p2, S0->nphi));
        if (S0->dim >= 2 && !S0->d_qy) NFCHK(dalloc(&S0->d_qy, S0->nphi));
        if (S0->dim == 3 && !S0->d_qz) NFCHK(dalloc(&S0->d_qz, S0->nphi));
    }
    if (R.form == CG_XCD && !pub_ready(T)) R.form = CG_FUSE3;
    if (R.form == CG_XCD) {
        const unsigned long long seq = ++T->pub_seq;
        NFCHK(launch_cg_xcd(S0, g, P.f3, x[0], seq));
        NFCHK(pub_wait(T, seq, &sc, nullptr, 0));
        if (sc.err != 3 && sc.err != 4) { T->last_xcd = 1; ++T->xcd_solves; HIPCHK(hipGetLastError()); return cg_result(T, g, CG_XCD, sc, its_out, res_out); }
        T->opt.cg_xcd = 0; ++T->xcd_refused; R.form = CG_FUSE3;
        if (sc.err == 4) { HIPCHK(hipStreamSynchronize(T->stream)); init(); }
        NFCHK(team_finalize(T, FIN_RHS, R.gcnt, 1, T->d_out, tol, maxit));
        memset(&sc, 0, sizeof sc);
    }
    if (R.form == CG_TEAM_VEC)
        for (double *slot : { T->d_partials + T->vec_cnt_pq, R.row1() + T->vec_cnt_rr }) HIPCHK(hipMemsetAsync(slot, 0, sizeof(double), T->stream));
    int launched = 0, rc = NF_OK;
    int batch = T->opt.cg_batch > 0 ? T->opt.cg_batch : (T->last_its[g] > 0 ? T->last_its[g] + 2 : 1), grow = 2;
    while (launched < maxit && rc == NF_OK) {
        const int nb = std::min(batch, maxit - launched);
        for (int it = 0; it < nb && rc == NF_OK; ++it) rc = cg_step(R, launched + it, T->cg_iter_total++);
        if (rc != NF_OK) break;
        launched += nb;
        rc = cg_stop_test(R, launched, &sc);
        if (rc != NF_OK || sc.done) break;
        batch = T->opt.cg_batch > 0 ? T->opt.cg_batch : (launched < 8 ? 1 : grow);
        if (launched >= 8) grow = std::min(64, 2 * grow);
    }
    NFCHK(rc);
    if (T->poisoned) return team_poison_result(T);
    if (sc.err == 2) return fail(NF_ERR_REMOTE, "another rank of the team reported an error during the CG solve of group %d; every rank stopped at iteration %d", g, sc.its);
    if (launched == 0) {
        HIPCHK(hipMemcpyAsync(&sc, T->d_cg, sizeof sc, hipMemcpyDeviceToHost, T->stream));
        HIPCHK(hipStreamSynchronize(T->stream));
    }
    if (P.fused)
        for (int i = 0; i < ns; ++i) {
            const double *plast = T->slabs[i]->d_p;
            if (R.form == CG_FUSE3 && sc.its >= 2 && ((sc.its - 1) & 1)) plast = T->slabs[i]->d_p2;
            hipLaunchKernelGGL(k_cg_flush, dim3(R.gcnt[i]), dim3(256), 0, T->stream, x[i], plast, T->slabs[i]->nphi, T->d_cg);
        }
    HIPCHK(hipGetLastError());
    if (T->profile) prof_collect(T);
    return cg_result(T, g, R.form, sc, its_out, res_out);
}

int nf_solve_group(nf_handle S, int g, const double *rhs_dev, double *phi_dev, double tol, int maxit, int *its, double *res)
{
    if (!S || !rhs_dev || !phi_dev || g < 0 || g >= S->ng) return fail(NF_ERR_ARG, "nf_solve_group: bad arguments");
    if (!S->built) return fail(NF_ERR_STATE, "nf_solve_group: call nf_build first");
    if (!team_is_single(S->team)) return fail(NF_ERR_STATE, "nf_solve_group works on an undivided mesh");
    HIPCHK(hipSetDevice(S->device));
    NFCHK(line_dict_prepare(S->team));
    return cg_solve(S->team, g, { rhs_dev }, { phi_dev }, tol, maxit, its, res);
}

int nf_build_diagonal_cache(nf_handle S)
{
    if (!S) return fail(NF_ERR_ARG, "null handle");
    nf_team *T = S->team;
    for (auto *X : T->slabs) if (!X->built) return fail(NF_ERR_STATE, "nf_build_diagonal_cache: call nf_build first");
    NFCHK(void_refuse(S, "nf_build_diagonal_cache"));
    if (S->k != 0 || S->m != 0) return NF_OK;
    bool valid = true, any_if = false;
    for (auto *X : T->slabs) { valid &= X->diag_valid; any_if |= X->if_lo || X->if_hi; }
    if (valid) return NF_OK;
    HIPCHK(hipSetDevice(S->device));
    {
        int lrc = NF_OK;
        for (auto *X : T->slabs) if (lrc == NF_OK && !X->d_Sinv) lrc = dalloc(&X->d_Sinv, (size_t)X->N * X->ng);
        NFCHK(team_verdict(T, lrc, "the edge-plane exchange of nf_build_diagonal_cache"));
    }
    for (int g = 0; g < S->ng; ++g) {
        if (any_if) {
            for (auto *X : T->slabs) {
                const long nl = X->nlines[2];
                hipLaunchKernelGGL(k_edge_a2, dim3((unsigned)((nl + 255) / 256)), dim3(256), 0, T->stream, make_geom(X), X->d_D + g * X->N, X->d_clo, X->d_chi, nl);
            }
            NFCHK(exchange_planes(T, 0, 0, T->stream));
        }
        for (auto *X : T->slabs) {
            const long N = X->N;
            hipLaunchKernelGGL(k_diag_cache, dim3((unsigned)((N + 255) / 256)), dim3(256), 0, T->stream, make_geom(X), X->d_D + g * N, X->d_Cd + g * N,
                               X->d_Sinv + g * N, N, X->if_lo ? X->d_rlo : (const double *)nullptr, X->if_hi ? X->d_rhi : (const double *)nullptr);
        }
        NFCHK(team_stream_wait(T, T->stream));
    }
    HIPCHK(hipGetLastError());
    for (auto *X : T->slabs) X->diag_valid = true;
    return NF_OK;
}
int nf_get_diagonal_cache(nf_handle S, int g, double *sinv_host)
{
// ... 2687 lines not shown
{
    if (!S || bytes < 16 || reps < 1 || !gbps) return fail(NF_ERR_ARG, "nf_time_device_copy: bad arguments");
    HIPCHK(hipSetDevice(S->device));
    hipStream_t st = S->team->stream;
    const long n2 = (long)(bytes / 16);
    nf_d2 *a = nullptr, *b = nullptr;
    NFCHK(dalloc(&a, (size_t)n2)); if (dalloc(&b, (size_t)n2) != NF_OK) { dfree(a); return NF_ERR_HIP; }
    (void)hipMemsetAsync(a, 0, (size_t)n2 * 16, st);
    hipEvent_t e0, e1; (void)hipEventCreate(&e0); (void)hipEventCreate(&e1);
    double best = 0.0; hipError_t e = hipSuccess;
    int ncu = 256; (void)hipDeviceGetAttribute(&ncu, hipDeviceAttributeMultiprocessorCount, S->device);
    const bool verbose = getenv("NEUTFEM_COPY_VERBOSE") != nullptr;
    struct V { int kind, per_cu; };
    const V vs[] = { {0, 16}, {0, 64}, {0, 256}, {0, 0}, {1, 16}, {1, 64}, {1, 256}, {1, 0}, {2, 64}, {2, 0}, {3, 0} };
    const int NV = (int)(sizeof vs / sizeof vs[0]);
    for (int variant = 0; variant < NV && e == hipSuccess; ++variant) {
        const V v = vs[variant];
        const int U = v.kind == 2 ? 8 : 4;
        const long full = (n2 + 256L * U - 1) / (256L * U);
        const int grid = (int)std::min<long>(v.per_cu ? (long)ncu * v.per_cu : full, full);
        auto once = [&]() {
            if (v.kind == 3) { (void)hipMemcpyAsync(b, a, (size_t)n2 * 16, hipMemcpyDeviceToDevice, st); return; }
            if (v.kind == 0) hipLaunchKernelGGL((k_copy<false, 4>), dim3(grid), dim3(256), 0, st, (const nf_d2 *)a, b, n2);
            else if (v.kind == 1) hipLaunchKernelGGL((k_copy<true, 4>), dim3(grid), dim3(256), 0, st, (const nf_d2 *)a, b, n2);
            else hipLaunchKernelGGL((k_copy<true, 8>), dim3(grid), dim3(256), 0, st, (const nf_d2 *)a, b, n2);
        };
        once();
        (void)hipEventRecord(e0, st);
        for (int i = 0; i < reps; ++i) once();
        (void)hipEventRecord(e1, st);
        e = hipEventSynchronize(e1);
        float ms = 0.f; (void)hipEventElapsedTime(&ms, e0, e1);
        const double gb = ms > 0.f ? 2.0 * (double)n2 * 16.0 * reps / (ms * 1e-3) / 1e9 : 0.0;
        if (verbose) fprintf(stderr, "[copy] variant %2d (%s, grid %d): %.0f GB/s\n", variant,
                             v.kind == 3 ? "hipMemcpyDtoD" : v.kind == 0 ? "plain, 4 in flight" : v.kind == 1 ? "nt, 4 in flight" : "nt, 8 in flight", v.kind == 3 ? 0 : grid, gb);
        if (e == hipSuccess) best = std::max(best, gb);
    }
    (void)hipEventDestroy(e0); (void)hipEventDestroy(e1);
    dfree(a); dfree(b);
    if (e != hipSuccess) return fail(NF_ERR_HIP, "nf_time_device_copy: %s", hipGetErrorString(e));
    *gbps = best;
    return NF_OK;
}

int nf_set_option(nf_handle S, const char *key, long value)
{
    if (!S || !key) return fail(NF_ERR_ARG, "nf_set_option: bad arguments");
    nf_team *T = S->team;
    const bool own = !strcmp(key, "transient_rebalance");
    NfOptions mine; unsigned fx = 0; std::string err;
    if (!nf_options_set(own ? mine : T->opt, key, value, &fx, &err)) return fail(NF_ERR_ARG, "%s", err.c_str());
    if (own) S->opt_tr_rebalance = (int)mine.transient_rebalance;
    if ((fx & NF_FX_RELINK) || ((fx & NF_FX_RELINK_MULTI) && T->nproc > 1)) T->linked_ready = false;
    return team_apply_table_effects(T, fx);
}
int nf_get_option(nf_handle S, const char *key, long *value)
{
    if (!S || !key || !value) return fail(NF_ERR_ARG, "nf_get_option: bad arguments");
    if (!nf_options_get(S->team->opt, key, value)) return fail(NF_ERR_ARG, "nf_get_option: unknown key %s", key);
    if (!strcmp(key, "transient_rebalance")) *value = S->opt_tr_rebalance;
    return NF_OK;
}

int nf_mem_info(int device, size_t *free_bytes, size_t *total_bytes)
{
    if (hipSetDevice(device) != hipSuccess) { (void)hipGetLastError(); return fail(NF_ERR_ARG, "nf_mem_info: device %d out of range", device); }
    size_t f = 0, t = 0;
    HIPCHK(hipMemGetInfo(&f, &t));
    if (free_bytes) *free_bytes = f;
    if (total_bytes) *total_bytes = t;
    return NF_OK;
}
int nf_dev_alloc(nf_handle S, size_t bytes, void **p)
{
    if (!S || !p) return fail(NF_ERR_ARG, "nf_dev_alloc: bad arguments");
    HIPCHK(hipSetDevice(S->device)); HIPCHK(hipMalloc(p, std::max<size_t>(bytes, 8))); return NF_OK;
}
int nf_dev_free(nf_handle S, void *p) { if (!S) return fail(NF_ERR_ARG, "null handle"); HIPCHK(hipSetDevice(S->device)); if (p) HIPCHK(hipFree(p)); return NF_OK; }
int nf_memcpy_h2d(nf_handle S, void *dst, const void *src, size_t bytes)
{
    if (!S || !dst || !src) return fail(NF_ERR_ARG, "nf_memcpy_h2d: bad arguments");
    HIPCHK(hipSetDevice(S->device)); HIPCHK(hipMemcpy(dst, src, bytes, hipMemcpyHostToDevice)); return NF_OK;
}
int nf_memcpy_d2h(nf_handle S, void *dst, const void *src, size_t bytes)
{
    if (!S || !dst || !src) return fail(NF_ERR_ARG, "nf_memcpy_d2h: bad arguments");
    HIPCHK(hipSetDevice(S->device)); HIPCHK(hipStreamSynchronize(S->team->stream)); HIPCHK(hipMemcpy(dst, src, bytes, hipMemcpyDeviceToHost)); return NF_OK;
}
int nf_synchronize(nf_handle S) { if (!S) return fail(NF_ERR_ARG, "null handle"); HIPCHK(hipSetDevice(S->device)); HIPCHK(hipStreamSynchronize(S->team->stream)); HIPCHK(hipDeviceSynchronize()); return NF_OK; }
void *nf_stream(nf_handle S) { return S ? (void *)S->team->stream : nullptr; }

extern "C" int nf_debug_xcd_buffer(void *h, double *out, int n, int coarse)
{
    nf_solver *S = (nf_solver *)h; if (!S || !S->team) return NF_ERR_ARG;
    nf_team *T = S->team;
    (void)coarse;
    if (!T->d_xpart) { for (int i = 0; i < n; ++i) out[i] = 0.0; return NF_OK; }
    HIPCHK(hipMemcpy(out, T->d_xpart, sizeof(double) * std::min(n, 512), hipMemcpyDeviceToHost));
    return NF_OK;
}
```

### neutfem_amd/csrc/nf_kernels.h

```cpp
#pragma once
#include <hip/hip_runtime.h>
#include "nf_outer.h"

#ifdef NF_STAMPS
#define NF_STAMP(buf, i) do { if (buf) (buf)[i] = (long long)__builtin_readcyclecounter(); } while (0)
#else
#define NF_STAMP(buf, i) do { } while (0)
#endif

#ifndef NF_SR_Z1_WAVES
#define NF_SR_Z1_WAVES 3
#endif
#ifndef NF_SR_Z2_WAVES
#define NF_SR_Z2_WAVES 4
#endif
#ifndef NF_STAGE_PLACE
#define NF_STAGE_PLACE 1
#endif

namespace nf {

struct CgScalars {
    double rr, pAp, alpha, beta, rr_new, tol_sq, rhs_norm, tol;
    int done, its, maxit;
// ... 72 lines not shown
    double s = 0.0;
    int i = threadIdx.x;
    if (threadIdx.x >= 256) return 0.0;
    for (; i + 7 * 256 < cnt; i += 8 * 256) {
        double v[8];
#pragma unroll
        for (int j = 0; j < 8; ++j) v[j] = p[i + j * 256];
#pragma unroll
        for (int j = 0; j < 8; ++j) s += v[j];
    }
    for (; i < cnt; i += 256) s += p[i];
    return s;
}
template <bool RAW> __device__ __forceinline__ void block_bar()
{
    if constexpr (RAW) { asm volatile("s_waitcnt lgkmcnt(0)" ::: "memory"); __builtin_amdgcn_s_barrier(); asm volatile("" ::: "memory"); }
    else __syncthreads();
}
template <bool RAW = false>
__device__ __forceinline__ double block_sum(double v, double *sred)
{
    v = wave_sum(v);
    const int lane = threadIdx.x & 63, w = threadIdx.x >> 6, nw = (blockDim.x + 63) >> 6;
    block_bar<RAW>();
    if (lane == 0) sred[w] = v;
    block_bar<RAW>();
    double s = 0.0;
    if (threadIdx.x == 0)
        for (int i = 0; i < nw; ++i) s += sred[i];
    return s;
}

__device__ __forceinline__ void block_sum3(double &a, double &b, double &c, double *sred)
{
    a = wave_sum(a); b = wave_sum(b); c = wave_sum(c);
    const int lane = threadIdx.x & 63, w = threadIdx.x >> 6, nw = (blockDim.x + 63) >> 6;
    __syncthreads();
    if (lane == 0) { sred[w] = a; sred[nw + w] = b; sred[2 * nw + w] = c; }
    __syncthreads();
    if (threadIdx.x == 0) {
        double sa = 0.0, sb = 0.0, sc = 0.0;
        for (int i = 0; i < nw; ++i) { sa += sred[i]; sb += sred[nw + i]; sc += sred[2 * nw + i]; }
        a = sa; b = sb; c = sc;
    }
}

struct PartSegs { int n; int off[16]; int cnt[16]; };
enum FinOp { FIN_RHS = 0, FIN_PAP = 1, FIN_RR = 2, FIN_SUM = 3 };

__device__ __forceinline__ int reduce_err(double total, double flag)
{
    return flag != 0.0 ? 2 : ((total - total) != 0.0 ? 1 : 0);
}
__device__ __forceinline__ void cg_logic(int op, const double *tot, int nq, CgScalars *cg, double *out, double tol, int maxit, double flag = 0.0)
{
    if (op == FIN_RHS) { cg->err = 0; }
    if (op != FIN_SUM) { const int e = reduce_err(tot[0], flag); if (e) { cg->err = e; cg->done = 1; if (op == FIN_RHS) { cg->rr = tot[0]; cg->its = 0; cg->pend = 0; } return; } }
    if (op == FIN_RHS) {
        cg->rr = tot[0];
        cg->rhs_norm = sqrt(tot[0]);
        cg->tol = tol;
        cg->tol_sq = tol * tol * cg->rhs_norm * cg->rhs_norm;
        cg->done = 0; cg->its = 0; cg->maxit = maxit; cg->pend = 0;
        cg->rr2[0] = tot[0]; cg->its2[0] = 0;
        if (maxit <= 0) cg->done = 1;
    } else if (op == FIN_PAP) {
        cg->pAp = tot[0];
        cg->pend = 0;
        if (fabs(tot[0]) < 1e-30) cg->done = 1;
        else cg->alpha = cg->rr / tot[0];
    } else if (op == FIN_RR) {
        cg->rr_new = tot[0];
        cg->its += 1;
        cg->pend = 1;
        if (tot[0] < cg->tol_sq) { cg->rr = tot[0]; cg->done = 1; }
        else {
            cg->beta = tot[0] / cg->rr;
            cg->rr = tot[0];
            if (cg->its >= cg->maxit) cg->done = 1;
        }
    } else {
        for (int q = 0; q < nq; ++q) out[q] = tot[q];
    }
}

__global__ __launch_bounds__(256) void k_finalize(int op, const double *__restrict__ partials, PartSegs segs, long stride,
                                                  int nq, CgScalars *__restrict__ cg, double *__restrict__ out,
                                                  double tol, int maxit, int reduce_only, double *__restrict__ red, const double *__restrict__ errsrc = nullptr)
{
    __shared__ double sred[4];
    if ((op == FIN_PAP || op == FIN_RR) && !reduce_only) { if (cg->done) return; }
    double tot[4] = { 0, 0, 0, 0 };
    for (int q = 0; q < nq; ++q) {
        double acc = 0.0;
        for (int sgi = 0; sgi < segs.n; ++sgi) {
            double s = strided_sum256(partials + q * stride + segs.off[sgi], segs.cnt[sgi]);
            s = block_sum(s, sred);
            acc += s;
        }
        tot[q] = acc;
    }
    if (threadIdx.x != 0) return;
    if (reduce_only) { for (int q = 0; q < nq; ++q) red[q] = tot[q]; if (errsrc) red[nq] = *errsrc; return; }
    cg_logic(op, tot, nq, cg, out, tol, maxit);
}
__global__ void k_cg_logic(int op, const double *__restrict__ red, int nq, CgScalars *__restrict__ cg, double *__restrict__ out,
                           double tol, int maxit, int with_flag)
{
    if (op == FIN_PAP || op == FIN_RR) { if (cg->done) return; }
    double tot[4] = { 0, 0, 0, 0 };
    for (int q = 0; q < nq; ++q) tot[q] = red[q];
    cg_logic(op, tot, nq, cg, out, tol, maxit, with_flag ? red[nq] : 0.0);
    if (with_flag == 2) out[nq] = red[nq];
}

__device__ __forceinline__ double strided_total(const double *p, int cnt, double *sred);
struct CgLean { CgScalars *st; const double *partials; int count; int par; int first; int flag_at; };
__device__ __forceinline__ double lean_total(const CgLean &lean, double *sred)
{
    return lean.count < 0 ? lean.partials[0] : strided_total(lean.partials, lean.count, sred);
}
__device__ __forceinline__ int lean_err(const CgLean &lean, double total)
{
    return reduce_err(total, lean.count < 0 ? lean.partials[1] : (lean.flag_at > 0 ? lean.partials[lean.flag_at] : 0.0));
}
__device__ __forceinline__ double strided_total(const double *p, int cnt, double *sred)
{
    double s = strided_sum256(p, cnt);
    s = block_sum(s, sred);
    if (threadIdx.x == 0) sred[0] = s;
    __syncthreads();
    s = sred[0];
    __syncthreads();
    return s;
}
struct LeanPre { double rr_old, tol_sq; int its_old, maxit; };
__device__ __forceinline__ LeanPre lean_preload(const CgLean &lean)
{
    const CgScalars *st = lean.st; const int qo = lean.par ^ 1;
    LeanPre p; p.rr_old = st->rr2[qo]; p.tol_sq = st->tol_sq; p.its_old = st->its2[qo]; p.maxit = st->maxit;
    return p;
}
__device__ __forceinline__ bool lean_rr_step(const CgLean &lean, const LeanPre &pre, bool writer, double *sred, double *beta_out)
{
    CgScalars *st = lean.st;
    const int q = lean.par;
    const double rr_new = lean_total(lean, sred);
    const int e = lean_err(lean, rr_new);
    if (e) {
        if (writer) { st->rr_new = rr_new; st->rr = rr_new; st->err = e; st->done = 1; }
        *beta_out = 0.0;
        return true;
    }
    const double rr_old = pre.rr_old;
    const int its_new = pre.its_old + 1;
    const bool conv = rr_new < pre.tol_sq;
    const bool stop = conv || its_new >= pre.maxit;
    const double beta = rr_new / rr_old;
    if (writer) {
        st->rr2[q] = rr_new; st->its2[q] = its_new;
        st->rr_new = rr_new; st->rr = rr_new; st->its = its_new; st->pend = 1;
        if (!conv) st->beta = beta;
        if (stop) st->done = 1;
    }
    *beta_out = beta;
// ... 286 lines not shown
}
__global__ void k_diag_cache(Geom G, const double *__restrict__ D, const double *__restrict__ Cd,
                             double *__restrict__ Sinv, long N, const double *__restrict__ nb_lo, const double *__restrict__ nb_hi)
{
    const long e = blockIdx.x * (long)blockDim.x + threadIdx.x;
    if (e >= N) return;
    const int ix = (int)(e % G.nx); const long r = e / G.nx; const int iy = (int)(r % G.ny); const int iz = (int)(r / G.ny);
    const long nxy = (long)G.nx * G.ny;
    double S = Cd[e];
    const double b2 = G.T0;
    for (int d = 0; d < G.dim; ++d) {
        const int c = d == 0 ? ix : d == 1 ? iy : iz;
        const int n = d == 0 ? G.nx : d == 1 ? G.ny : G.nz;
        const long sl = d == 0 ? 1 : d == 1 ? G.nx : nxy;
        double a2, a1, b2n, b1n;
        cell_a(G, d, ix, iy, iz, D[e], a2, a1);
        double Alo = a2, Ahi = a2;
        if (c > 0) {
            int jx = ix - (d == 0), jy = iy - (d == 1), jz = iz - (d == 2);
            cell_a(G, d, jx, jy, jz, D[e - sl], b2n, b1n); Alo += b2n;
        } else if (d == 2 && nb_lo) Alo += nb_lo[e % nxy];
        else if (G.dir_lo[d]) Alo += dirichlet_term(G, d, ix, iy, iz, D[e]);
        if (c + 1 < n) {
            int jx = ix + (d == 0), jy = iy + (d == 1), jz = iz + (d == 2);
            cell_a(G, d, jx, jy, jz, D[e + sl], b2n, b1n); Ahi += b2n;
        } else if (d == 2 && nb_hi) Ahi += nb_hi[e % nxy];
        else if (G.dir_hi[d]) Ahi += dirichlet_term(G, d, ix, iy, iz, D[e]);
        if (fabs(G.T0 * Alo) > 1e-14) S += b2 / Alo;
        if (fabs(G.T0 * Ahi) > 1e-14) S += b2 / Ahi;
    }
    Sinv[e] = fabs(S) > 1e-14 ? 1.0 / S : 0.0;
}

typedef double nf_d2 __attribute__((ext_vector_type(2)));
template <bool NT = false>
__device__ __forceinline__ void ld2(const double *p, long i, bool ok, bool vec, double &a, double &b, bool ok2)
{
    if (vec) {
        nf_d2 v = { 0.0, 0.0 };
        if (ok) v = NT ? __builtin_nontemporal_load(reinterpret_cast<const nf_d2 *>(p + i)) : *reinterpret_cast<const nf_d2 *>(p + i);
        a = v.x; b = v.y;
    } else if (NT) { a = ok ? __builtin_nontemporal_load(p + i) : 0.0; b = ok2 ? __builtin_nontemporal_load(p + i + 1) : 0.0; }
    else { a = ok ? p[i] : 0.0; b = ok2 ? p[i + 1] : 0.0; }
}
template <bool NT>
__device__ __forceinline__ double ldg(const double *p) { return NT ? __builtin_nontemporal_load(p) : *p; }
template <bool NT> __device__ __forceinline__ double ldo(const double *p, unsigned byte_off)
{
    const double *q = reinterpret_cast<const double *>(reinterpret_cast<const char *>(p) + byte_off);
    return NT ? __builtin_nontemporal_load(q) : *q;
}
__device__ __forceinline__ void sto(double *p, unsigned byte_off, double v) { *reinterpret_cast<double *>(reinterpret_cast<char *>(p) + byte_off) = v; }

struct CgFuse { double *p; const double *r; double *xsol; double *pout; };

struct LineDict { const int *id = nullptr; int pitch = 0; };
struct LineFp { unsigned long long lo, hi; };
__device__ __forceinline__ void line_span(int d, long line, int nx, int ny, int nz, long &base, long &sl, int &n)
{
    const long nxy = (long)nx * ny;
    if (d == 0) { n = nx; base = line * nx; sl = 1; }
    else if (d == 1) { n = ny; base = (line / nx) * nxy + line % nx; sl = nx; }
    else { n = nz; base = line; sl = nxy; }
}
__device__ __forceinline__ void fp_mix(unsigned long long &a, unsigned long long &b, double v)
{
    const unsigned long long u = (unsigned long long)__double_as_longlong(v);
    a ^= u; a *= 0xff51afd7ed558ccdull; a ^= a >> 33;
    b = ((b << 27) | (b >> 37)) + u; b *= 0xc4ceb9fe1a85ec53ull; b ^= b >> 31;
}
__global__ void k_line_fp(int d, int nx, int ny, int nz, const double *__restrict__ L, const double *__restrict__ DR, const double *__restrict__ D0,
                          const double *__restrict__ Cd, long nlines, int bits, LineFp *__restrict__ out)
{
    const long line = blockIdx.x * (long)blockDim.x + threadIdx.x;
    if (line >= nlines) return;
    long base, sl; int n;
    line_span(d, line, nx, ny, nz, base, sl, n);
    unsigned long long a = 0x9e3779b97f4a7c15ull, b = 0xd1b54a32d192ed03ull;
    fp_mix(a, b, D0[line]);
    for (int c = 0; c < n; ++c) {
        const long e = base + c * sl;
        fp_mix(a, b, L[e]); fp_mix(a, b, DR[e]);
        if (Cd) fp_mix(a, b, Cd[e]);
    }
    if (bits < 64) { b = 0; a &= bits <= 0 ? 0ull : (~0ull >> (64 - bits)); }
    else if (bits < 128) b &= bits == 64 ? 0ull : (~0ull >> (128 - bits));
    out[line].lo = a; out[line].hi = b;
}
__global__ void k_line_verify(int d, int nx, int ny, int nz, const double *__restrict__ L, const double *__restrict__ DR, const double *__restrict__ D0,
                              const double *__restrict__ Cd, long nlines, const int *__restrict__ id, const int *__restrict__ rep, int *__restrict__ mism)
{
    const long line = blockIdx.x * (long)blockDim.x + threadIdx.x;
    if (line >= nlines) return;
    const long other = rep[id[line]];
    if (other == line) return;
    long base, sl, ob, osl; int n;
    line_span(d, line, nx, ny, nz, base, sl, n);
    line_span(d, other, nx, ny, nz, ob, osl, n);
    bool same = __double_as_longlong(D0[line]) == __double_as_longlong(D0[other]);
    for (int c = 0; c < n; ++c) {
        const long e = base + c * sl, o = ob + c * osl;
        same = same && __double_as_longlong(L[e]) == __double_as_longlong(L[o]) && __double_as_longlong(DR[e]) == __double_as_longlong(DR[o]);
        if (Cd) same = same && __double_as_longlong(Cd[e]) == __double_as_longlong(Cd[o]);
    }
    if (!same) atomicAdd(mism, 1);
}
__global__ void k_line_gather(int d, int nx, int ny, int nz, const double *__restrict__ L, const double *__restrict__ DR, const double *__restrict__ Cd,
                              const int *__restrict__ rep, int nrows, int pitch, double *__restrict__ tL, double *__restrict__ tR, double *__restrict__ tC)
{
    const long i = blockIdx.x * (long)blockDim.x + threadIdx.x;
    if (i >= (long)nrows * pitch) return;
    const int row = (int)(i / pitch), c = (int)(i % pitch);
    long base, sl; int n;
    line_span(d, rep[row], nx, ny, nz, base, sl, n);
    const bool in = c < n; const long e = base + c * sl;
    tL[i] = in ? L[e] : 0.0; tR[i] = in ? DR[e] : 0.0;
    if (tC) tC[i] = in ? Cd[e] : 0.0;
}

template <int K, int NCH, bool VEC, int NB, class Mid = NoMid, bool DPPS = false, bool NT = false, bool DICT = false>
__device__ __forceinline__ double schur_x_task(const ModeArgs &ma, const Geom &G, const double *__restrict__ L, const double *__restrict__ DR,
                                               const double *__restrict__ D0, int nx, int ny, long nlines, int lpl_log2, int first,
                                               long task, int lane, bool active, bool fuse, double f_alpha, double f_beta, const CgFuse &fz, Mid mid = Mid(),
                                               const LineDict &ld = LineDict())
{
    static_assert(K == 2, "two cells per lane and chunk");
    static_assert(!DICT || (NB == 0 && NT), "line tables: next to the streaming RT0-P0 instantiations only");
    const int LPL = 1 << lpl_log2, LPW = 64 >> lpl_log2;
    const int li = lane & (LPL - 1), sub = lane >> lpl_log2;
    const long line = task * LPW + sub;
    const bool lv = active && line < nlines;
    const long base = lv ? line * nx : 0;
    const int iy = lv ? (int)(line % ny) : 0, iz = lv ? (int)(line / ny) : 0;
    long cbase = base;
    if (DICT) cbase = lv ? (long)((unsigned)ld.id[line] * (unsigned)ld.pitch) : 0;
    constexpr bool NTC = NT && !DICT;
    double xm[NB + 1][NCH][K], yo[NB + 1][NCH][K], Ls[NCH][K], Rs[NCH][K], w[NCH][K], xL[NCH][K], xR[NCH][K], ic[NCH][K];
    double rq[NB + 1][NCH][K], sq[NB + 1][NCH][K], dq[NB > 0 ? NCH : 1][K];
    double *pw = fz.pout ? fz.pout : fz.p;
#pragma unroll
    for (int ch = 0; ch < NCH; ++ch) {
        const int c0 = (ch * LPL + li) * K;
        const bool ok = lv && c0 < nx, ok2 = lv && c0 + 1 < nx;
        ld2<NTC>(L, cbase + c0, ok, VEC, Ls[ch][0], Ls[ch][1], ok2);
        ld2<NTC>(DR, cbase + c0, ok, VEC, Rs[ch][0], Rs[ch][1], ok2);
#pragma unroll
        for (int q = 0; q <= NB; ++q) {
            ld2<NT>(ma.x[q], base + c0, ok, VEC, xm[q][ch][0], xm[q][ch][1], ok2);
            if (DICT && first) ld2<false>(ma.Cd[q], cbase + c0, ok, VEC, yo[q][ch][0], yo[q][ch][1], ok2);
            else ld2<NT>(first ? ma.Cd[q] : ma.y[q], base + c0, ok, VEC, yo[q][ch][0], yo[q][ch][1], ok2);
            if (fuse) {
                const long mo = (ma.x[q] - fz.p) + base + c0;
                ld2<NT>(fz.r, mo, ok, VEC, rq[q][ch][0], rq[q][ch][1], ok2);
                ld2<NT>(fz.xsol, mo, ok, VEC, sq[q][ch][0], sq[q][ch][1], ok2);
            }
        }
        if (NB > 0) ld2<NT>(ma.D, base + c0, ok, VEC, dq[NB > 0 ? ch : 0][0], dq[NB > 0 ? ch : 0][1], ok2);
    }
    if (mid(f_alpha, f_beta)) return 0.0;
#pragma unroll
    for (int ch = 0; ch < NCH; ++ch) {
        const int c0 = (ch * LPL + li) * K;
        const bool ok = lv && c0 < nx, ok2 = lv && c0 + 1 < nx;
        if (fuse) {
#pragma unroll
            for (int q = 0; q <= NB; ++q) {
                const long mo = (ma.x[q] - fz.p) + base + c0;
                const double s0 = fma(f_alpha, xm[q][ch][0], sq[q][ch][0]), s1 = fma(f_alpha, xm[q][ch][1], sq[q][ch][1]);
                xm[q][ch][0] = fma(f_beta, xm[q][ch][0], rq[q][ch][0]); xm[q][ch][1] = fma(f_beta, xm[q][ch][1], rq[q][ch][1]);
                if (VEC) {
                    if (ok) { *reinterpret_cast<double2 *>(fz.xsol + mo) = make_double2(s0, s1);
                              *reinterpret_cast<double2 *>(pw + mo) = make_double2(xm[q][ch][0], xm[q][ch][1]); }
                } else {
                    if (ok) { fz.xsol[mo] = s0; pw[mo] = xm[q][ch][0]; }
                    if (ok2) { fz.xsol[mo + 1] = s1; pw[mo + 1] = xm[q][ch][1]; }
                }
            }
        }
#pragma unroll
        for (int j = 0; j < K; ++j) {
            double pl = 0.0, pr = 0.0;
            ic[ch][j] = 0.0;
            if (NB > 0) {
                const double dd = dq[NB > 0 ? ch : 0][j];
                const bool okj = j == 0 ? ok : ok2;
                ic[ch][j] = okj ? dd / geom_factor(G, 0, c0 + j, iy, iz) : 0.0;
#pragma unroll
                for (int l = 0; l < NB; ++l) { const double gx = ma.Gc[l] * xm[l + 1][ch][j]; pl += ma.eL[l] * gx; pr += ma.eR[l] * gx; }
            }
            xL[ch][j] = xm[0][ch][j] + pl; xR[ch][j] = xm[0][ch][j] - pr;
        }
    }
    const double d0 = lv ? D0[line] : 0.0;
    const double z0 = __shfl(-xL[0][0], 0, LPL);
    double carry = z0;
#pragma unroll
    for (int ch = 0; ch < NCH; ++ch) {
        double xn = DPPS ? lane_above(xL[ch][0]) : __shfl_down(xL[ch][0], 1, LPL);
        double xc = 0.0;
        if (ch + 1 < NCH) xc = __shfl(xL[ch + 1 < NCH ? ch + 1 : ch][0], 0, LPL);
        if (li == LPL - 1) xn = xc;
        double t[K];
#pragma unroll
        for (int j = 0; j < K; ++j) t[j] = xR[ch][j] - (j + 1 < K ? xL[ch][j + 1 < K ? j + 1 : j] : xn);
        double A = 1.0, B = 0.0;
#pragma unroll
        for (int j = 0; j < K; ++j) { B = t[j] - Ls[ch][j] * B; A = -Ls[ch][j] * A; }
        if (DPPS) scan_maps_up(A, B, LPL, lane);
        else for (int d = 1; d < LPL; d <<= 1) {
            const double Ap = __shfl_up(A, d, LPL), Bp = __shfl_up(B, d, LPL);
            if (li >= d) { B = A * Bp + B; A = A * Ap; }
        }
        const double Ae = DPPS ? lane_below(A) : __shfl_up(A, 1, LPL), Be = DPPS ? lane_below(B) : __shfl_up(B, 1, LPL);
        double z = li == 0 ? carry : Ae * carry + Be;
#pragma unroll
        for (int j = 0; j < K; ++j) { z = t[j] - Ls[ch][j] * z; w[ch][j] = z * Rs[ch][j]; }
        if (ch + 1 < NCH) carry = __shfl(z, LPL - 1, LPL);
    }
    double ucarry = 0.0, dot = 0.0;
#pragma unroll
    for (int ch = NCH - 1; ch >= 0; --ch) {
        double Ln = DPPS ? lane_above(Ls[ch][0]) : __shfl_down(Ls[ch][0], 1, LPL);
        double Lc = 0.0;
        if (ch + 1 < NCH) Lc = __shfl(Ls[ch + 1 < NCH ? ch + 1 : ch][0], 0, LPL);
        if (li == LPL - 1) Ln = Lc;
        double Lup[K];
#pragma unroll
        for (int j = 0; j < K; ++j) Lup[j] = j + 1 < K ? Ls[ch][j + 1 < K ? j + 1 : j] : Ln;
        double A = 1.0, B = 0.0;
#pragma unroll
        for (int j = K - 1; j >= 0; --j) { B = w[ch][j] - Lup[j] * B; A = -Lup[j] * A; }
        if (DPPS) scan_maps_down(A, B, LPL, lane);
        else for (int d = 1; d < LPL; d <<= 1) {
            const double Ap = __shfl_down(A, d, LPL), Bp = __shfl_down(B, d, LPL);
            if (li + d < LPL) { B = A * Bp + B; A = A * Ap; }
        }
        const double Ae = DPPS ? lane_above(A) : __shfl_down(A, 1, LPL), Be = DPPS ? lane_above(B) : __shfl_down(B, 1, LPL);
        double u = li == LPL - 1 ? ucarry : Ae * ucarry + Be;
        double uv[K];
#pragma unroll
        for (int j = K - 1; j >= 0; --j) { u = w[ch][j] - Lup[j] * u; uv[j] = u; }
        if (ch > 0) ucarry = __shfl(uv[0], 0, LPL);
        double ulo = DPPS ? lane_below(uv[K - 1]) : __shfl_up(uv[K - 1], 1, LPL);
        double wprev = 0.0;
        if (ch > 0) wprev = __shfl(w[ch > 0 ? ch - 1 : 0][K - 1], LPL - 1, LPL);
        if (li == 0) ulo = (ch == 0 ? z0 * d0 : wprev) - Ls[ch][0] * uv[0];
        double yv[NB + 1][K];
#pragma unroll
        for (int j = 0; j < K; ++j) {
            const double lo = j == 0 ? ulo : uv[j > 0 ? j - 1 : 0];
            yv[0][j] = (first ? yo[0][ch][j] * xm[0][ch][j] : yo[0][ch][j]) + ma.Ta * (uv[j] - lo);
            dot += xm[0][ch][j] * yv[0][j];
#pragma unroll
            for (int l = 0; l < NB; ++l) {
                const double v = ma.Gc[l] * xm[l + 1][ch][j] * ma.iM[l] * ic[ch][j] - (ma.eL[l] * lo + ma.eR[l] * uv[j]);
                yv[l + 1][j] = (first ? yo[l + 1][ch][j] * xm[l + 1][ch][j] : yo[l + 1][ch][j]) + ma.Ta * ma.Gc[l] * v;
                dot += xm[l + 1][ch][j] * yv[l + 1][j];
            }
        }
        const int c0 = (ch * LPL + li) * K;
#pragma unroll
        for (int q = 0; q <= NB; ++q) {
            if (VEC) { if (lv && c0 < nx) *reinterpret_cast<double2 *>(ma.y[q] + base + c0) = make_double2(yv[q][0], yv[q][K - 1]); }
            else {
#pragma unroll
                for (int j = 0; j < K; ++j) if (lv && c0 + j < nx) ma.y[q][base + c0 + j] = yv[q][j];
            }
        }
    }
    return dot;
}

template <int K, int NCH, bool VEC, int NB, bool NT = false, bool DICT = false>
__global__ __launch_bounds__(256) void k_schur_x(ModeArgs ma0, ModeTab mt, Geom G, const double *__restrict__ L, const double *__restrict__ DR,
                                                 const double *__restrict__ D0, int nx, int ny, long nlines, int lpl_log2,
                                                 int first, int last, double *__restrict__ partials,
                                                 const CgScalars *__restrict__ cg, CgFuse fz, CgLean lean, LineDict ld = LineDict())
{
    __shared__ double sred[4];
    if (cg && cg->done) return;
    const ModeArgs ma = select_mode(ma0, mt, blockIdx.y, NB + 1);
    const bool lean_on = lean.st && !lean.first;
    const bool fuse = fz.p != nullptr && (lean.st ? lean_on : cg->its > 0);
    const double alpha0 = fuse ? cg->alpha : 0.0, beta0 = (fuse && !lean.st) ? cg->beta : 0.0;
    LeanPre pre = { 0.0, 0.0, 0, 0 };
    if (lean_on) pre = lean_preload(lean);
    bool stopped = false;
    auto mid = [&](double &fa, double &fb) -> bool {
        (void)fa;
        if (lean_on) stopped = lean_rr_step(lean, pre, blockIdx.x == 0 && blockIdx.y == 0 && threadIdx.x == 0, sred, &fb);
        return stopped;
    };
    unsigned bx = blockIdx.x;
    if ((first & 2) && gridDim.x % 8 == 0) bx = (blockIdx.x % 8) * (gridDim.x / 8) + blockIdx.x / 8;
    const double dot = schur_x_task<K, NCH, VEC, NB, decltype(mid), false, NT, DICT>(ma, G, L, DR, D0, nx, ny, nlines, lpl_log2, first & 1, (long)bx * 4 + (threadIdx.x >> 6),
                                                                           threadIdx.x & 63, true, fuse, alpha0, beta0, fz, mid, ld);
    if (stopped) return;
    if (last && partials) {
        const double s = block_sum(dot, sred);
        if (threadIdx.x == 0) partials[(long)blockIdx.y * gridDim.x + bx] = s;
    }
}

struct SlabArgs {
    int if_lo, if_hi, mode, xcd;
    int fold; const double *rlo, *rhi, *sinv_lo, *sinv_hi;
    int wsmin;
    int noacc; const double *yadd;
    const double *alo, *ahi, *ulo, *uhi;
    double *clo, *chi;
    double *jz;
    double *jzb;
    int nfa, ni, amode[9];
    Cg1 sr; double *sr_r; const double *sr_q; double *sr_part; long sr_stride;
};
enum : unsigned { SV_FUSE = 1, SV_NT = 2, SV_ZW = 4, SV_SR = 8, SV_DICT = 16, SV_STAGE = 32, SV_ALL = 63 };
constexpr bool schur_s_legal(int SEG, int DIR, bool SLAB, int NB, unsigned V)
{
    const bool p0 = NB == 0, s8 = p0 && SEG == 8;
    const unsigned admits = (SLAB && p0 ? SV_FUSE : 0) | (s8 ? SV_NT : 0) | (!SLAB && p0 ? SV_ZW : 0) | (SLAB && s8 && DIR == 2 ? SV_SR : 0) | (!SLAB && (V & SV_NT) ? SV_DICT : 0)
                            | (!SLAB && s8 && (V & SV_NT) && (V & SV_DICT) ? SV_STAGE : 0);
    return (SEG == 4 || SEG == 8 || (p0 && (SEG == 16 || SEG == 32))) && (DIR == 2 || (DIR == 1 && !SLAB)) && NB >= 0 && NB <= 2 && !(V & ~admits);
}
struct StageCtx {
    const double *buf = nullptr, *next = nullptr;
    const int *next_id = nullptr;
    int id = 0;
};
template <bool NT, bool REDO = false>
__device__ __forceinline__ void stage_issue(const double *buf, const double *src, int n, long sl, int TX)
{
    typedef __attribute__((address_space(1))) const void *gptr_t;
    typedef __attribute__((address_space(3))) void *lptr_t;
    int lane = threadIdx.x & 63; const int w = __builtin_amdgcn_readfirstlane(threadIdx.x >> 6), nw = blockDim.x >> 6;
    if (REDO) asm volatile("" : "+v"(lane));
    const int lpr = TX >> 1, rpp = 64 / lpr;
    const int rl = lane / lpr, cl = lane % lpr;
    const char *dst = reinterpret_cast<const char *>(buf);
    for (int p = w, np = (n + rpp - 1) / rpp; p < np; p += nw) {
        const int r = p * rpp + rl;
        if (r < n) __builtin_amdgcn_global_load_lds((gptr_t)(src + (long)r * sl + 2 * cl), (lptr_t)(dst + p * 1024), 16, 0, NT ? 2 : 0);
    }
}
template <int SEG, int DIR, bool SLAB, int NB, unsigned V = 0, class Mid = NoMid, bool XC = false, bool FULL = false>
__device__ __forceinline__ double schur_s_tile(const ModeArgs &ma, const Geom &G, const double *__restrict__ L, const double *__restrict__ DR,
                                               const double *__restrict__ D0, int n, long sl, long outer_stride, int nx, int TX, int NSEG,
                                               unsigned bx, unsigned by, unsigned bz, unsigned gy, int tid, bool act, double *sm,
                                               const SlabArgs &sa, const CgFuse &fz, bool fuse, bool fro, double f_alpha, double f_beta, bool acc,
// ... 1113 lines not shown
    __shared__ double sred[4];
    double s = 0.0;
    for (long i = blockIdx.x * 256L + threadIdx.x; i < n; i += gridDim.x * 256L) {
        double b = rhs[i];
        if constexpr (MASK) if (void_entry(vm, i, n)) b = 0.0;
        x[i] = 0.0; r[i] = b; p[i] = b; s += b * b;
    }
    s = block_sum(s, sred);
    if (threadIdx.x == 0) partials[blockIdx.x] = s;
}
template <bool MASK>
__global__ __launch_bounds__(256) void k_cg_update(double *__restrict__ x, double *__restrict__ r,
                                                   const double *__restrict__ p, const double *__restrict__ q, long n,
                                                   const CgScalars *__restrict__ cg, double *__restrict__ partials, VoidMask vm)
{
    __shared__ double sred[4];
    if (cg->done) return;
    const double alpha = cg->alpha;
    double s = 0.0;
    for (long i = blockIdx.x * 256L + threadIdx.x; i < n; i += gridDim.x * 256L) {
        x[i] = fma(alpha, p[i], x[i]);
        double rn = r[i] - alpha * q[i];
        if constexpr (MASK) if (void_entry(vm, i, n)) rn = 0.0;
        r[i] = rn; s += rn * rn;
    }
    s = block_sum(s, sred);
    if (threadIdx.x == 0) partials[blockIdx.x] = s;
}
template <bool MASK>
__global__ __launch_bounds__(256) void k_cg_rupdate(double *__restrict__ r, const double *__restrict__ q, long n,
                                                    const CgScalars *__restrict__ cg, double *__restrict__ partials, CgLean lean, VoidMask vm)
{
    __shared__ double sred[4];
    if (cg->done) return;
    double alpha;
    if (lean.st) {
        const double pq = lean_total(lean, sred);
        const int e = lean_err(lean, pq);
        if (e) { if (blockIdx.x == 0 && threadIdx.x == 0) { lean.st->pAp = pq; lean.st->err = e; lean.st->done = 1; } return; }
        const bool brk = fabs(pq) < 1e-30;
        alpha = brk ? 0.0 : lean.st->rr2[lean.par] / pq;
        if (blockIdx.x == 0 && threadIdx.x == 0) { lean.st->pAp = pq; lean.st->pend = 0; if (brk) lean.st->done = 1; else lean.st->alpha = alpha; }
        if (brk) return;
    } else alpha = cg->alpha;
    double s = 0.0;
    for (long i = blockIdx.x * 256L + threadIdx.x; i < n; i += gridDim.x * 256L) {
        double rn = r[i] - alpha * q[i];
        if constexpr (MASK) if (void_entry(vm, i, n)) rn = 0.0;
        r[i] = rn; s += rn * rn;
    }
    s = block_sum(s, sred);
    if (threadIdx.x == 0) partials[blockIdx.x] = s;
}
__global__ void k_cg_flush(double *__restrict__ x, const double *__restrict__ p, long n, const CgScalars *__restrict__ cg)
{
    if (!cg->pend) return;
    const double alpha = cg->alpha;
    for (long i = blockIdx.x * 256L + threadIdx.x; i < n; i += gridDim.x * 256L) x[i] = fma(alpha, p[i], x[i]);
}
__global__ __launch_bounds__(256) void k_cg_pupdate(double *__restrict__ p, const double *__restrict__ r, long n,
                                                    const CgScalars *__restrict__ cg)
{
    if (cg->done) return;
    const double beta = cg->beta;
    for (long i = blockIdx.x * 256L + threadIdx.x; i < n; i += gridDim.x * 256L) p[i] = fma(beta, p[i], r[i]);
}

__global__ __launch_bounds__(256) void k_fission(const double *__restrict__ Mf, const double *__restrict__ phi, int ng,
                                                 long n, double *__restrict__ tf, double *__restrict__ partials,
                                                 const double *__restrict__ w, long nw)
{
    __shared__ double sred[4];
    double s = 0.0;
    for (long i = blockIdx.x * 256L + threadIdx.x; i < n; i += gridDim.x * 256L) {
        double v = 0.0;
        for (int g = 0; g < ng; ++g) v += Mf[g * n + i] * phi[g * n + i];
        tf[i] = v;
        if (!w) s += v; else if (i < nw) s += w[i] * v;
    }
    s = block_sum(s, sred);
    if (threadIdx.x == 0) partials[blockIdx.x] = s;
}
struct ScatterArgs { const double *M[64]; int ng; };
template <bool SRC>
__global__ __launch_bounds__(256) void k_group_rhs(ScatterArgs sa, int g, const double *__restrict__ chi,
                                                   const double *__restrict__ tf, double inv_k,
                                                   const double *__restrict__ phi_new, const double *__restrict__ phi_old,
                                                   const double *__restrict__ sinv, double *__restrict__ out, long n, long ncell,
                                                   double *__restrict__ x0 = nullptr, double *__restrict__ r0 = nullptr, double *__restrict__ p0 = nullptr,
                                                   double *__restrict__ partials = nullptr, const double *__restrict__ q = nullptr)
{
    __shared__ double sred[4];
    double s2 = 0.0;
    for (long i = blockIdx.x * 256L + threadIdx.x; i < n; i += gridDim.x * 256L) {
        double v;
        if (n == ncell) v = inv_k * (chi[i] * tf[i]);
        else { const double cv = chi[i % ncell] * inv_k; v = fabs(cv) < 1e-14 ? 0.0 : cv * tf[i]; }
        for (int gp = 0; gp < sa.ng; ++gp) {
            if (gp == g || !sa.M[gp]) continue;
            const double *ph = gp < g ? phi_new : phi_old;
            v += sa.M[gp][i] * ph[gp * n + i];
        }
        if constexpr (SRC) v += q[i];
        out[i] = sinv ? sinv[i] * v : v;
        if (r0) { x0[i] = 0.0; r0[i] = v; p0[i] = v; s2 += v * v; }
    }
    if (r0) {
        s2 = block_sum(s2, sred);
        if (threadIdx.x == 0) partials[blockIdx.x] = s2;
    }
}
// ... 1961 lines not shown
```

### neutfem_amd/csrc/nf_options.h

```cpp
#pragma once
#include <climits>
#include <cstring>
#include <string>

constexpr long NF_OPT_RED_GRID = 1024;

struct NfOptions {
    long xy_overlap = 1, xy_overlap_max_cells = 6L << 20;
    long xchg_comm = 0;
    long cg_single_reduce = -1, cg_single_reduce_max_cells = 1L << 40;
    long endpoint_weights = 1;
    long vec_reduce = 1;
    long host_pub = 1;
    long prof_every = 8;
    long cg_batch = 0;
    long nt_loads = 1, nt_min_cells = 8000000;
    long cg_fuse = 1;
    long xcd = -1;
    long outer_dev = 1;
    long cg_lean = 1, cg_lean_grid = NF_OPT_RED_GRID;
    long cg_lean_max_cells = 4L << 20;
    long sep_fold = 1;
    long s_tx = 0, s_seg = 0, s_wsmin = 0;
    long split_dot = 1;
    long s_long_dirs = 3;
    long s_long_min_y = 255;
    long line_dict = -1, line_dict_dirs = 7, line_dict_fp_bits = 128, line_dict_max_bytes = 512L * 1024;
    long s_long = -1, s_long_min = 256;
    long c_early = -1;
    long s_stage = -1, s_stage_grid = 0;
    long tile_full = -1;
    long cg_fuse3 = 1, cg_fuse3_max_cells = 400000;
    long sens_grid = NF_OPT_RED_GRID;
    long kin_grid = NF_OPT_RED_GRID;
    long cg_xcd = 1, keff_xcd = 1, cg_xcd_id = 0, cg_xcd_groups = 32, cg_xcd_min_cells = 2000, cg_xcd_max_cells = 28000;
    long resident = 1, resident_lds = 1, resident_serial = 1, resident_two_sided = 1, resident_max_dofs = 2500, resident_serial_max_dofs = 5120;
    long direct_max_dofs = 6000;
    long transient_rebalance = 1;
};

enum : unsigned {
    NF_FX_RELINK = 1,
    NF_FX_RELINK_MULTI = 2,
    NF_FX_DICT = 4,
    NF_FX_REGIME = 8
};
enum NfCopy { NF_COPY_NONE, NF_COPY_SOLVE, NF_COPY_PASS };
enum NfNorm {
    NF_BOOL,
    NF_CLAMP,
    NF_MASK,
    NF_POW2,
    NF_ATLEAST,
    NF_RAW,
    NF_INT,
    NF_RETIRED
};
struct NfOptionRow { const char *key; long NfOptions::*field; NfNorm norm; long lo, hi; NfCopy copy; unsigned effects; const char *err; long NfOptions::*also; };

inline const NfOptionRow *nf_option_rows(int *n)
{
#define NF_ROW(k, ...) { #k, &NfOptions::k, __VA_ARGS__ }
    static const NfOptionRow rows[] = {
        NF_ROW(s_tx, NF_POW2, 8, 64, NF_COPY_PASS, NF_FX_RELINK_MULTI | NF_FX_REGIME, "nf_set_option: s_tx must be 0 (auto), 8, 16, 32 or 64", nullptr),
        NF_ROW(s_seg, NF_POW2, 4, 32, NF_COPY_PASS, NF_FX_RELINK_MULTI | NF_FX_REGIME, "nf_set_option: s_seg must be 0 (auto), 4, 8, 16 or 32", nullptr),
        { "s_pair", nullptr, NF_RETIRED, 0, 0, NF_COPY_NONE, 0, nullptr, nullptr },
        { "x_two_phase", nullptr, NF_RETIRED, 0, 0, NF_COPY_NONE, 0, nullptr, nullptr },
        NF_ROW(s_wsmin, NF_CLAMP, 0, 100000, NF_COPY_PASS, 0, nullptr, nullptr),
        NF_ROW(vec_reduce, NF_BOOL, 0, 1, NF_COPY_PASS, 0, nullptr, nullptr),
// ... 1 lines not shown
        NF_ROW(cg_single_reduce_max_cells, NF_CLAMP, 0, LONG_MAX, NF_COPY_SOLVE, NF_FX_RELINK, nullptr, nullptr),
        NF_ROW(endpoint_weights, NF_BOOL, 0, 1, NF_COPY_SOLVE, NF_FX_RELINK, nullptr, nullptr),
        NF_ROW(xchg_comm, NF_BOOL, 0, 1, NF_COPY_NONE, NF_FX_RELINK_MULTI, nullptr, nullptr),
        NF_ROW(xy_overlap, NF_BOOL, 0, 1, NF_COPY_PASS, 0, nullptr, nullptr),
        NF_ROW(xy_overlap_max_cells, NF_CLAMP, 0, LONG_MAX, NF_COPY_PASS, 0, nullptr, nullptr),
        NF_ROW(split_dot, NF_CLAMP, 0, 2, NF_COPY_PASS, 0, nullptr, nullptr),
        NF_ROW(s_long, NF_CLAMP, -1, 1, NF_COPY_PASS, NF_FX_REGIME, nullptr, nullptr),
        NF_ROW(s_long_dirs, NF_MASK, 0, 3, NF_COPY_PASS, NF_FX_REGIME, nullptr, nullptr),
        NF_ROW(s_long_min_y, NF_CLAMP, 1, 1000000, NF_COPY_PASS, NF_FX_REGIME, nullptr, nullptr),
        NF_ROW(s_long_min, NF_CLAMP, 1, 1000000, NF_COPY_PASS, NF_FX_REGIME, nullptr, nullptr),
        NF_ROW(c_early, NF_CLAMP, -1, 2, NF_COPY_PASS, 0, nullptr, nullptr),
        NF_ROW(s_stage, NF_CLAMP, -1, 1, NF_COPY_PASS, 0, nullptr, nullptr),
        NF_ROW(tile_full, NF_CLAMP, -1, 1, NF_COPY_PASS, 0, nullptr, nullptr),
        NF_ROW(s_stage_grid, NF_CLAMP, 0, 1L << 20, NF_COPY_PASS, 0, nullptr, nullptr),
        NF_ROW(line_dict, NF_CLAMP, -1, 1, NF_COPY_PASS, NF_FX_DICT, nullptr, nullptr),
        NF_ROW(line_dict_dirs, NF_MASK, 0, 7, NF_COPY_PASS, NF_FX_DICT, nullptr, nullptr),
        NF_ROW(line_dict_max_bytes, NF_CLAMP, 0, 1L << 30, NF_COPY_PASS, NF_FX_DICT, nullptr, nullptr),
        NF_ROW(line_dict_fp_bits, NF_CLAMP, 0, 128, NF_COPY_PASS, NF_FX_DICT, nullptr, nullptr),
        NF_ROW(cg_batch, NF_INT, 0, 0, NF_COPY_SOLVE, 0, nullptr, nullptr),
        NF_ROW(cg_fuse, NF_BOOL, 0, 1, NF_COPY_SOLVE, 0, nullptr, nullptr),
        NF_ROW(xcd, NF_MASK, -1, 7, NF_COPY_PASS, 0, nullptr, nullptr),
        NF_ROW(host_pub, NF_BOOL, 0, 1, NF_COPY_PASS, 0, nullptr, nullptr),
        NF_ROW(prof_every, NF_ATLEAST, 1, 0, NF_COPY_PASS, 0, "prof_every must be >= 1", nullptr),
        NF_ROW(nt_loads, NF_BOOL, 0, 1, NF_COPY_PASS, NF_FX_REGIME, nullptr, nullptr),
        NF_ROW(nt_min_cells, NF_RAW, 0, 0, NF_COPY_PASS, NF_FX_REGIME, nullptr, nullptr),
        NF_ROW(outer_dev, NF_BOOL, 0, 1, NF_COPY_SOLVE, 0, nullptr, nullptr),
        NF_ROW(cg_lean, NF_BOOL, 0, 1, NF_COPY_SOLVE, 0, nullptr, nullptr),
        NF_ROW(sep_fold, NF_BOOL, 0, 1, NF_COPY_SOLVE, 0, nullptr, nullptr),
        NF_ROW(cg_lean_max_cells, NF_RAW, 0, 0, NF_COPY_SOLVE, 0, nullptr, nullptr),
        NF_ROW(resident, NF_BOOL, 0, 1, NF_COPY_SOLVE, 0, nullptr, nullptr),
        NF_ROW(resident_lds, NF_BOOL, 0, 1, NF_COPY_SOLVE, 0, nullptr, nullptr),
        NF_ROW(resident_serial, NF_BOOL, 0, 1, NF_COPY_SOLVE, 0, nullptr, nullptr),
        NF_ROW(resident_two_sided, NF_BOOL, 0, 1, NF_COPY_SOLVE, 0, nullptr, nullptr),
        NF_ROW(resident_max_dofs, NF_RAW, 0, 5120, NF_COPY_SOLVE, 0, nullptr, &NfOptions::resident_serial_max_dofs),
        NF_ROW(resident_serial_max_dofs, NF_RAW, 0, 0, NF_COPY_SOLVE, 0, nullptr, nullptr),
        NF_ROW(direct_max_dofs, NF_CLAMP, 0, 8192, NF_COPY_SOLVE, 0, nullptr, nullptr),
        NF_ROW(cg_fuse3, NF_BOOL, 0, 1, NF_COPY_SOLVE, 0, nullptr, nullptr),
        NF_ROW(cg_xcd, NF_BOOL, 0, 1, NF_COPY_SOLVE, 0, nullptr, nullptr),
        NF_ROW(keff_xcd, NF_BOOL, 0, 1, NF_COPY_SOLVE, 0, nullptr, nullptr),
        NF_ROW(cg_xcd_min_cells, NF_RAW, 0, 0, NF_COPY_SOLVE, 0, nullptr, nullptr),
        NF_ROW(cg_xcd_max_cells, NF_RAW, 0, 0, NF_COPY_SOLVE, 0, nullptr, nullptr),
        NF_ROW(cg_xcd_id, NF_MASK, 0, 15, NF_COPY_SOLVE, 0, nullptr, nullptr),
        NF_ROW(cg_xcd_groups, NF_CLAMP, 1, 64, NF_COPY_SOLVE, 0, nullptr, nullptr),
        NF_ROW(cg_fuse3_max_cells, NF_RAW, 0, 0, NF_COPY_SOLVE, 0, nullptr, nullptr),
        NF_ROW(cg_lean_grid, NF_CLAMP, 1, 1024, NF_COPY_SOLVE, 0, nullptr, nullptr),
        NF_ROW(sens_grid, NF_CLAMP, 1, 65536, NF_COPY_PASS, 0, nullptr, nullptr),
        NF_ROW(kin_grid, NF_CLAMP, 1, NF_OPT_RED_GRID, NF_COPY_PASS, 0, nullptr, nullptr),
        NF_ROW(transient_rebalance, NF_BOOL, 0, 1, NF_COPY_NONE, 0, nullptr, nullptr),
    };
#undef NF_ROW
    *n = (int)(sizeof rows / sizeof rows[0]);
    return rows;
}
inline const NfOptionRow *nf_option_find(const char *key)
{
    int n = 0; const NfOptionRow *rows = nf_option_rows(&n);
    for (int i = 0; i < n; ++i) if (!strcmp(key, rows[i].key)) return rows + i;
    return nullptr;
}

inline bool nf_options_set(NfOptions &o, const char *key, long value, unsigned *effects, std::string *err)
{
    const NfOptionRow *r = nf_option_find(key);
    if (!r) { *err = std::string("nf_set_option: unknown key ") + key; return false; }
    long v = value;
    switch (r->norm) {
    case NF_BOOL: v = value != 0; break;
    case NF_CLAMP: v = value < r->lo ? r->lo : value > r->hi ? r->hi : value; break;
    case NF_MASK: v = r->lo < 0 && value < 0 ? -1 : value & r->hi; break;
    case NF_POW2: if (value != 0 && (value < r->lo || value > r->hi || (value & (value - 1)))) { *err = r->err; return false; } break;
    case NF_ATLEAST: if (value < r->lo) { *err = r->err; return false; } break;
    case NF_RAW: if (r->also) o.*r->also = value < r->hi ? value : r->hi; break;
    case NF_INT: v = (int)value; break;
    case NF_RETIRED: break;
    }
    if (r->field) o.*r->field = v;
    *effects = r->effects;
    return true;
}
inline bool nf_options_get(const NfOptions &o, const char *key, long *value)
{
    const NfOptionRow *r = nf_option_find(key);
    if (!r) return false;
    *value = r->field ? o.*r->field : 0;
    return true;
}
inline unsigned nf_options_copy(NfOptions &dst, const NfOptions &src, bool same_mesh_kind)
{
    int n = 0; const NfOptionRow *rows = nf_option_rows(&n);
    unsigned fx = 0;
    for (int i = 0; i < n; ++i) {
        const NfOptionRow &r = rows[i];
        if (r.copy == NF_COPY_NONE || (r.copy == NF_COPY_PASS && !same_mesh_kind) || dst.*r.field == src.*r.field) continue;
        dst.*r.field = src.*r.field; fx |= r.effects;
    }
    return fx & (NF_FX_DICT | NF_FX_REGIME);
}
```

Measured before the change: 5.126 outer-iters/s.

## Batch CG solution-vector updates through a ring of search directions

Keeps the last M search directions in a device ring buffer and records per-iteration alphas in a small device history, so the fused x-sweep skips reading and writing x_sol on most CG iterations. Every M-th iteration it applies the accumulated updates from the older directions in one pass, and the final flush applies any pending ones. This is meant to cut per-iteration memory traffic on the large grid, at the cost of (M-1) extra direction-sized buffers, extra loads on the apply iteration, more kernel instantiations, and bookkeeping that has to stay correct.

```diff
diff --git a/neutfem_amd/csrc/neutfem_hip.hip b/neutfem_amd/csrc/neutfem_hip.hip
--- a/neutfem_amd/csrc/neutfem_hip.hip
+++ b/neutfem_amd/csrc/neutfem_hip.hip
@@ -4,6 +4,7 @@
 #include "nf_line_groups.h"
 #include "nf_options.h"
 #include "nf_small_eig.h"
+#include "nf_xsol_ring.h"
 
 #include <dlfcn.h>
 #include <unistd.h>
@@ -112,6 +113,7 @@
     bool rccl_reduce = false;
     double *d_partials = nullptr; long partial_stride = 0, slab_cap = 0;
     CgScalars *d_cg = nullptr;
+    double *d_ah = nullptr;
     double *d_out = nullptr;
     double *d_red = nullptr;
     double *d_errsrc = nullptr;
@@ -187,6 +189,7 @@
     double *d_phi = nullptr, *d_raw = nullptr;
     double *d_p0 = nullptr, *d_p1 = nullptr;
     double *d_tf = nullptr, *d_rhs = nullptr, *d_r = nullptr, *d_p = nullptr, *d_q = nullptr;
+    double *d_ring = nullptr; int ring_m = 0; bool ring_refused = false;
     double *d_p2 = nullptr, *d_qy = nullptr, *d_qz = nullptr;
     bool raw_valid = false, raw_is_diag = false;
     double *d_qsrc = nullptr;
@@ -330,6 +333,7 @@
     T->slab_cap = cap; T->partial_stride = cap * (long)T->slabs.size();
     NFCHK(dalloc(&T->d_partials, (size_t)T->partial_stride * 4));
     if (!T->d_cg) NFCHK(dalloc(&T->d_cg, 1));
+    if (!T->d_ah) { NFCHK(dalloc(&T->d_ah, 8)); HIPCHK(hipMemset(T->d_ah, 0, 8 * sizeof(double))); }
     if (!T->d_out) NFCHK(dalloc(&T->d_out, 8));
     if (!T->d_red) NFCHK(dalloc(&T->d_red, 8));
     if (!T->d_errsrc) { NFCHK(dalloc(&T->d_errsrc, 1)); HIPCHK(hipMemset(T->d_errsrc, 0, sizeof(double))); }
@@ -360,7 +364,7 @@
     if (T->comm && g_rccl.CommDestroy) g_rccl.CommDestroy(T->comm);
     if (T->d_xcd) (void)hipFree(T->d_xcd);
     dfree(T->d_xpart);
-    dfree(T->d_partials); dfree(T->d_cg); dfree(T->d_out); dfree(T->d_red); dfree(T->d_errsrc); dfree(T->d_vec); dfree(T->d_ost); dfree(T->d_hist); dfree(T->d_hist_cg); dfree(T->d_rout);
+    dfree(T->d_partials); dfree(T->d_cg); dfree(T->d_ah); dfree(T->d_out); dfree(T->d_red); dfree(T->d_errsrc); dfree(T->d_vec); dfree(T->d_ost); dfree(T->d_hist); dfree(T->d_hist_cg); dfree(T->d_rout);
     if (T->h_pub) (void)hipHostFree(T->h_pub);
     if (T->comm_stream) { (void)hipStreamSynchronize(T->comm_stream); (void)hipStreamDestroy(T->comm_stream); }
     if (T->y_stream) { (void)hipStreamSynchronize(T->y_stream); (void)hipStreamDestroy(T->y_stream); }
@@ -513,7 +517,7 @@
     dfree(S->d_Wlo); dfree(S->d_Whi);
     dfree(S->d_Jz); dfree(S->d_Jzb); dfree(S->d_ctlo); dfree(S->d_cthi); dfree(S->d_elo); dfree(S->d_ehi); dfree(S->d_relo); dfree(S->d_rehi);
     dfree(S->d_phi); dfree(S->d_raw); dfree(S->d_p0); dfree(S->d_p1);
-    dfree(S->d_tf); dfree(S->d_rhs); dfree(S->d_r); dfree(S->d_p); dfree(S->d_q); dfree(S->d_p2); dfree(S->d_qy); dfree(S->d_qz);
+    dfree(S->d_tf); dfree(S->d_rhs); dfree(S->d_r); dfree(S->d_p); dfree(S->d_q); dfree(S->d_p2); dfree(S->d_qy); dfree(S->d_qz); dfree(S->d_ring);
     dfree(S->d_qsrc); dfree(S->d_modes[0]); dfree(S->d_modes[1]);
     dfree(S->d_gamma); dfree(S->d_gpt_w); dfree(S->d_gpt_sc);
     if (T) {
@@ -931,14 +935,21 @@
     CgLean lean = {};
     CgLean lean_z1 = {};
     Cg1 cg1 = {};
+    bool ring = false; CgFuse ringfz = {}; int xb = XB_NOW; const double *pnew = nullptr;
 };
 struct PassCg {
     const CgScalars *cg = nullptr; CgFuse fuse = {}; CgLean lean = {}, lean_z1 = {}; Cg1 cg1 = {};
     bool zw_dot = false;
     hipStream_t stream = nullptr;
     bool noacc = false; const double *yadd = nullptr;
+    int xb = XB_NOW;
 };
-static PassCg pass_cg(const ApplyCg &A, const nf_solver *S, int i) { return { A.cg, A.fused ? CgFuse{ S->d_p, S->d_r, (*A.xsol)[i] } : CgFuse{}, A.lean, A.lean_z1, A.cg1 }; }
+static PassCg pass_cg(const ApplyCg &A, const nf_solver *S, int i)
+{
+    PassCg P = { A.cg, A.fused ? CgFuse{ S->d_p, S->d_r, (*A.xsol)[i] } : CgFuse{}, A.lean, A.lean_z1, A.cg1 };
+    if (A.ring) { P.fuse = A.ringfz; P.xb = A.xb; }
+    return P;
+}
 struct SegPlan { int rc = NF_OK, SEG = 0, NSEG = 0, TX = 0, nparts = 0; dim3 grid, block; size_t lds = 0; };
 static SegPlan seg_plan(const nf_solver *S, int d, int zmode);
 static int launch_s(const nf_solver *S, int d, int g, const ModeArgs &ma, const Geom &G, int last, double *partials, const PassCg &P, int *nparts, int zmode);
@@ -1058,12 +1069,12 @@
 {
     PartSegs ps = segs_for(T, counts);
     if (!T->rccl_reduce) {
-        hipLaunchKernelGGL(k_finalize, dim3(1), dim3(256), 0, T->stream, op, T->d_partials, ps, T->partial_stride, nq, T->d_cg, out, tol, maxit, 0, T->d_red, (const double *)nullptr);
+        hipLaunchKernelGGL(k_finalize, dim3(1), dim3(256), 0, T->stream, op, T->d_partials, ps, T->partial_stride, nq, T->d_cg, out, tol, maxit, 0, T->d_red, (const double *)nullptr, T->d_ah);
     } else {
         hipLaunchKernelGGL(k_finalize, dim3(1), dim3(256), 0, T->stream, op, T->d_partials, ps, T->partial_stride, nq, T->d_cg, out, tol, maxit, 1, T->d_red, (const double *)T->d_errsrc);
         TRACE_COMM("rank %d allreduce finalize op=%d count=%d poisoned=%d", T->rank, op, nq + 1, (int)T->poisoned);
         NCCLCHK(g_rccl.AllReduce(T->d_red, T->d_red, (size_t)nq + 1, NCCL_DOUBLE, NCCL_SUM, T->comm, T->stream));
-        hipLaunchKernelGGL(k_cg_logic, dim3(1), dim3(1), 0, T->stream, op, T->d_red, nq, T->d_cg, out, tol, maxit, want_flag ? 2 : 1);
+        hipLaunchKernelGGL(k_cg_logic, dim3(1), dim3(1), 0, T->stream, op, T->d_red, nq, T->d_cg, out, tol, maxit, want_flag ? 2 : 1, T->d_ah);
     }
     return NF_OK;
 }
@@ -1162,10 +1173,12 @@
 }
 template <unsigned N, class F> static bool with_index(unsigned key, F &&f) { return with_index(key, f, std::make_integer_sequence<unsigned, N>()); }
 
-constexpr bool schur_x_legal(int NCH, bool VEC, int NB, bool NT, bool DICT)
+static const int X_BATCH_MAX_NCH = 8;
+constexpr bool schur_x_legal(int NCH, bool VEC, int NB, bool NT, bool DICT, int XB = XB_NOW)
 {
     return NCH >= 1 && NCH <= (NB == 0 ? 32 : 8) && (NCH & (NCH - 1)) == 0 && NB >= 0 && NB <= 2
-        && (!NT || (VEC && NB == 0)) && (!DICT || (NT && NCH <= X_DICT_MAX_NCH));
+        && (!NT || (VEC && NB == 0)) && (!DICT || (NT && NCH <= X_DICT_MAX_NCH))
+        && XB >= XB_NOW && XB <= XB_APPLY && (XB == XB_NOW || (NB == 0 && NCH <= X_BATCH_MAX_NCH));
 }
 struct XPlan { int lpl_log2 = 0, NCH = 0; unsigned grid = 0; bool vec = false, nt = false, xcd = false, dict = false; };
 static XPlan x_plan(const nf_solver *S)
@@ -1194,16 +1207,16 @@
     ModeArgs ma = ma0; if (da.on) ma.Cd[0] = da.C;
     const double *L = da.on ? da.L : S->d_L[0] + g * S->N, *DR = da.on ? da.DR : S->d_DR[0] + g * S->N, *D0 = S->d_D0[0] + g * S->nlines[0];
     int lg = 0; while ((1 << lg) < xp.NCH) ++lg;
-    const unsigned key = ((((unsigned)lg * 3 + (unsigned)S->nb) * 2 + xp.vec) * 2 + xp.nt) * 2 + xp.dict;
-    const bool hit = with_index<6 * 3 * 8>(key, [&](auto i) {
+    const unsigned key = (((((unsigned)P.xb * 6 + (unsigned)lg) * 3 + (unsigned)S->nb) * 2 + xp.vec) * 2 + xp.nt) * 2 + xp.dict;
+    const bool hit = with_index<3 * 6 * 3 * 8>(key, [&](auto i) {
         constexpr unsigned I = decltype(i)::value;
-        constexpr int NCH = 1 << (I / 24), NB = I / 8 % 3; constexpr bool VEC = I & 4, NT = I & 2, DICT = I & 1;
-        if constexpr (!schur_x_legal(NCH, VEC, NB, NT, DICT)) return false;
-        else hipLaunchKernelGGL((k_schur_x<2, NCH, VEC, NB, NT, DICT>), gr, dim3(256), 0, S->team->stream, ma, mt, G, L, DR, D0, S->nx, S->ny, S->nlines[0], xp.lpl_log2,
+        constexpr int XB = I / 144, NCH = 1 << (I / 24 % 6), NB = I / 8 % 3; constexpr bool VEC = I & 4, NT = I & 2, DICT = I & 1;
+        if constexpr (!schur_x_legal(NCH, VEC, NB, NT, DICT, XB)) return false;
+        else hipLaunchKernelGGL((k_schur_x<2, NCH, VEC, NB, NT, DICT, XB>), gr, dim3(256), 0, S->team->stream, ma, mt, G, L, DR, D0, S->nx, S->ny, S->nlines[0], xp.lpl_log2,
                                 first, last, partials, P.cg, fz, P.lean, da.ld);
         return true;
     });
-    return hit ? NF_OK : fail(NF_ERR_ARG, "k_schur_x: no instantiation for NCH = %d, NB = %d, vec %d, nt %d, dict %d", xp.NCH, S->nb, xp.vec, xp.nt, xp.dict);
+    return hit ? NF_OK : fail(NF_ERR_ARG, "k_schur_x: no instantiation for NCH = %d, NB = %d, vec %d, nt %d, dict %d, xb %d", xp.NCH, S->nb, xp.vec, xp.nt, xp.dict, P.xb);
 }
 
 struct ChunkPlan { bool ok = false; int NS = 0, TX = 0; size_t lds = 0; };
@@ -1580,7 +1593,8 @@
             if (xy_all && !S->d_qy) NFCHK(dalloc(&S->d_qy, S->nphi));
             {
                 double *part = (want_dot && (last || split)) ? T->d_partials + i * T->slab_cap + totals[i] : nullptr;
-                const ModeArgs ma = mode_args(S, g, d, 0, xs[i], ys[i]);
+                const double *xin = d > 0 && A.pnew ? A.pnew : xs[i];
+                const ModeArgs ma = mode_args(S, g, d, 0, xin, ys[i]);
                 int np = 0;
                 PassCg P = pass_cg(A, S, i); P.zw_dot = split;
                 if (d == 0) NFCHK(launch_x(S, g, ma, G, last || split, part, P, &np));
@@ -1589,7 +1603,7 @@
                     NFCHK(launch_s(S, 2, g, ma, G, last, part, P, &np, 2));
                 } else if (d == 1 && xy_all) {
                     P.stream = T->y_stream; P.noacc = true;
-                    NFCHK(launch_s(S, 1, g, mode_args(S, g, 1, 0, xs[i], S->d_qy), G, 0, nullptr, P, &np, 0));
+                    NFCHK(launch_s(S, 1, g, mode_args(S, g, 1, 0, xin, S->d_qy), G, 0, nullptr, P, &np, 0));
                 } else NFCHK(launch_s(S, d, g, ma, G, last || split, part, P, &np, 0));
                 if (part) totals[i] += np;
             }
@@ -1786,8 +1800,21 @@
     CgForm form = CG_CLASSIC; Fuse3Plan f3; int gru = 0;
     bool fused = false; int reductions = 0;
     bool lean() const { return form == CG_XCD || form == CG_FUSE3 || form == CG_LEAN; }
+    int xsol_batch = 1;
 };
+static const int XSOL_BATCH_AUTO = 4;
+static CgPlan cg_plan_form(const nf_team *T);
 static CgPlan cg_plan(const nf_team *T)
+{
+    CgPlan P = cg_plan_form(T); const nf_solver *S0 = T->slabs[0];
+    if (P.form != CG_FUSED || !team_is_single(T) || !x_fuses(S0) || S0->nb != 0 || S0->ring_refused) return P;
+    const int nch = x_plan(S0).NCH;
+    if (nch < 1 || nch > X_BATCH_MAX_NCH) return P;
+    const long o = T->opt.xsol_batch;
+    P.xsol_batch = o < 0 ? (S0->N > T->opt.cg_lean_max_cells ? XSOL_BATCH_AUTO : 1) : (int)std::min<long>(std::max<long>(o, 1), NF_XSOL_RING_MAX);
+    return P;
+}
+static CgPlan cg_plan_form(const nf_team *T)
 {
     CgPlan P; const nf_solver *S0 = T->slabs[0]; const bool single = team_is_single(T);
     P.fused = T->opt.cg_fuse != 0 && (single || S0->nloc == 1);
@@ -1848,9 +1875,9 @@
     const bool split = split_dot(T, cg, lean);
     bool any_if = false; for (auto *X : T->slabs) any_if |= X->if_lo || X->if_hi;
     const bool xy_all = xy_overlap(T, any_if, false);
-    char tmp[288];
-    snprintf(tmp, sizeof tmp, "{\"in_cg\": %d, \"form\": \"%s\", \"slab\": %d, \"fused\": %d, \"lean\": %d, \"single_reduce\": %d, \"split_dot\": %d, \"xy_overlap\": %d, \"passes\": [",
-             cg ? 1 : 0, cg ? CG_FORM_NAME[cp.form] : "", slab ? 1 : 0, fused ? 1 : 0, lean ? 1 : 0, sr ? 1 : 0, split ? 1 : 0, xy_all ? 1 : 0);
+    char tmp[320];
+    snprintf(tmp, sizeof tmp, "{\"in_cg\": %d, \"form\": \"%s\", \"xsol_batch\": %d, \"slab\": %d, \"fused\": %d, \"lean\": %d, \"single_reduce\": %d, \"split_dot\": %d, \"xy_overlap\": %d, \"passes\": [",
+             cg ? 1 : 0, cg ? CG_FORM_NAME[cp.form] : "", cg ? cp.xsol_batch : 1, slab ? 1 : 0, fused ? 1 : 0, lean ? 1 : 0, sr ? 1 : 0, split ? 1 : 0, xy_all ? 1 : 0);
     std::string js = tmp;
     for (int d = 0; d < S->dim; ++d) {
         const bool last = d == S->dim - 1, want_dot = cg && (last || split);
@@ -1881,6 +1908,8 @@
     std::vector<const double *> ps; std::vector<double *> qs;
     std::vector<int> gcnt, acnt, cnt3;
     bool any_if = false;
+    int M = 1;
+    double *slot(int s) const { nf_solver *S = T->slabs[0]; return s == 0 ? S->d_p : S->d_ring + (size_t)(s - 1) * S->nphi; }
     double *row1() const { return T->d_partials + T->partial_stride; }
     double *vec_rr() const { return T->d_vec + T->vec_stride; }
     int chk(int rc) const { return team_poison(T, rc, form == CG_TEAM_VEC) ? rc : NF_OK; }
@@ -1894,6 +1923,16 @@
     if (R.form == CG_TEAM_SR) A.cg1 = Cg1{ T->d_red, T->d_cg, index };
     if (R.form == CG_TEAM_VEC) A.lean_z1 = CgLean{ T->d_cg, R.vec_rr(), T->vec_cnt_rr, index & 1, first, T->vec_cnt_rr };
     if (R.form == CG_TEAM_LEAN) A.lean_z1 = CgLean{ T->d_cg, T->d_red + 2, -1, index & 1, first };
+    if (R.M > 1) {
+        const int rd = nf_ring_read(index, R.M), wr = nf_ring_write(index, R.M);
+        const NfRingBatch B = nf_ring_apply(index, R.M);
+        A.ring = true; A.xb = index == 0 ? XB_NOW : B.n ? XB_APPLY : XB_SKIP; A.pnew = R.slot(wr);
+        A.ringfz = CgFuse{ R.slot(rd), T->slabs[0]->d_r, R.x[0], wr == rd ? nullptr : R.slot(wr) };
+        if (B.n) {
+            A.ringfz.nold = B.n - 1; A.ringfz.a0 = B.u[0].alpha; A.ringfz.ah = T->d_ah;
+            for (int i = 0; i + 1 < B.n; ++i) A.ringfz.old[i] = R.slot(B.u[i].slot);
+        }
+    }
     return A;
 }
 static int cg_step_fuse3(CgRun &R, int index)
@@ -1918,7 +1957,11 @@
     int ra = NF_OK;
     if (T->nproc > 1 && T->rank == T->inject_rank && global_it == T->inject_iter)
         { ra = fail(NF_ERR_HIP, "injected failure on rank %d at CG iteration %ld (NEUTFEM_INJECT_FAIL)", T->rank, global_it); TRACE_COMM("rank %d INJECT at %ld", T->rank, global_it); }
-    else if (!T->poisoned) ra = team_schur_apply(T, R.g, R.ps, R.qs, true, cg_apply_args(R, index), &R.acnt, &R.cnt3);
+    else if (!T->poisoned) {
+        const ApplyCg A = cg_apply_args(R, index);
+        if (A.ring) R.ps[0] = A.ringfz.p;
+        ra = team_schur_apply(T, R.g, R.ps, R.qs, true, A, &R.acnt, &R.cnt3);
+    }
     NFCHK(R.chk(ra));
     if (T->poisoned && R.any_if) {
         if (T->xchg_in_apply == 0) { (void)hipEventRecord(T->ev_z1, T->stream); (void)hipStreamWaitEvent(T->comm_stream, T->ev_z1, 0); }
@@ -2010,6 +2053,14 @@
         if (S0->dim >= 2 && !S0->d_qy) NFCHK(dalloc(&S0->d_qy, S0->nphi));
         if (S0->dim == 3 && !S0->d_qz) NFCHK(dalloc(&S0->d_qz, S0->nphi));
     }
+    if (P.xsol_batch > 1) {
+        if (S0->ring_m != P.xsol_batch) {
+            dfree(S0->d_ring); S0->ring_m = 0;
+            if (hipMalloc((void **)&S0->d_ring, (size_t)(P.xsol_batch - 1) * S0->nphi * sizeof(double)) == hipSuccess) S0->ring_m = P.xsol_batch;
+            else { (void)hipGetLastError(); S0->d_ring = nullptr; S0->ring_refused = true; }
+        }
+        if (S0->ring_m == P.xsol_batch) R.M = P.xsol_batch;
+    }
     if (R.form == CG_XCD && !pub_ready(T)) R.form = CG_FUSE3;
     if (R.form == CG_XCD) {
         const unsigned long long seq = ++T->pub_seq;
@@ -2042,11 +2093,17 @@
         HIPCHK(hipMemcpyAsync(&sc, T->d_cg, sizeof sc, hipMemcpyDeviceToHost, T->stream));
         HIPCHK(hipStreamSynchronize(T->stream));
     }
-    if (P.fused)
+    if (P.fused && R.M > 1) {
+        const NfRingBatch B = nf_ring_pending(sc.its, sc.pend, R.M);
+        FlushRing fr; memset(&fr, 0, sizeof fr); fr.n = B.n; fr.ah = T->d_ah;
+        for (int j = 0; j < B.n; ++j) { fr.alpha[j] = B.u[j].alpha; fr.p[j] = R.slot(B.u[j].slot); }
+        if (B.n > 0) hipLaunchKernelGGL(k_cg_flush, dim3(R.gcnt[0]), dim3(256), 0, T->stream, x[0], (const double *)nullptr, S0->nphi, T->d_cg, fr);
+    } else if (P.fused)
         for (int i = 0; i < ns; ++i) {
             const double *plast = T->slabs[i]->d_p;
             if (R.form == CG_FUSE3 && sc.its >= 2 && ((sc.its - 1) & 1)) plast = T->slabs[i]->d_p2;
-            hipLaunchKernelGGL(k_cg_flush, dim3(R.gcnt[i]), dim3(256), 0, T->stream, x[i], plast, T->slabs[i]->nphi, T->d_cg);
+            FlushRing fr; memset(&fr, 0, sizeof fr); fr.n = -1;
+            hipLaunchKernelGGL(k_cg_flush, dim3(R.gcnt[i]), dim3(256), 0, T->stream, x[i], plast, T->slabs[i]->nphi, T->d_cg, fr);
         }
     HIPCHK(hipGetLastError());
     if (T->profile) prof_collect(T);
@@ -4840,6 +4897,7 @@
     if (!nf_options_set(own ? mine : T->opt, key, value, &fx, &err)) return fail(NF_ERR_ARG, "%s", err.c_str());
     if (own) S->opt_tr_rebalance = (int)mine.transient_rebalance;
     if ((fx & NF_FX_RELINK) || ((fx & NF_FX_RELINK_MULTI) && T->nproc > 1)) T->linked_ready = false;
+    if (!strcmp(key, "xsol_batch")) { HIPCHK(hipSetDevice(T->device)); for (auto *X : T->slabs) { dfree(X->d_ring); X->ring_m = 0; X->ring_refused = false; } }
     return team_apply_table_effects(T, fx);
 }
 int nf_get_option(nf_handle S, const char *key, long *value)
diff --git a/neutfem_amd/csrc/nf_kernels.h b/neutfem_amd/csrc/nf_kernels.h
--- a/neutfem_amd/csrc/nf_kernels.h
+++ b/neutfem_amd/csrc/nf_kernels.h
@@ -148,7 +148,7 @@
 {
     return flag != 0.0 ? 2 : ((total - total) != 0.0 ? 1 : 0);
 }
-__device__ __forceinline__ void cg_logic(int op, const double *tot, int nq, CgScalars *cg, double *out, double tol, int maxit, double flag = 0.0)
+__device__ __forceinline__ void cg_logic(int op, const double *tot, int nq, CgScalars *cg, double *out, double tol, int maxit, double flag = 0.0, double *ah = nullptr)
 {
     if (op == FIN_RHS) { cg->err = 0; }
     if (op != FIN_SUM) { const int e = reduce_err(tot[0], flag); if (e) { cg->err = e; cg->done = 1; if (op == FIN_RHS) { cg->rr = tot[0]; cg->its = 0; cg->pend = 0; } return; } }
@@ -164,7 +164,7 @@
         cg->pAp = tot[0];
         cg->pend = 0;
         if (fabs(tot[0]) < 1e-30) cg->done = 1;
-        else cg->alpha = cg->rr / tot[0];
+        else { cg->alpha = cg->rr / tot[0]; if (ah) ah[cg->its & 7] = cg->alpha; }
     } else if (op == FIN_RR) {
         cg->rr_new = tot[0];
         cg->its += 1;
@@ -182,7 +182,8 @@
 
 __global__ __launch_bounds__(256) void k_finalize(int op, const double *__restrict__ partials, PartSegs segs, long stride,
                                                   int nq, CgScalars *__restrict__ cg, double *__restrict__ out,
-                                                  double tol, int maxit, int reduce_only, double *__restrict__ red, const double *__restrict__ errsrc = nullptr)
+                                                  double tol, int maxit, int reduce_only, double *__restrict__ red, const double *__restrict__ errsrc = nullptr,
+                                                  double *__restrict__ ah = nullptr)
 {
     __shared__ double sred[4];
     if ((op == FIN_PAP || op == FIN_RR) && !reduce_only) { if (cg->done) return; }
@@ -198,15 +199,15 @@
     }
     if (threadIdx.x != 0) return;
     if (reduce_only) { for (int q = 0; q < nq; ++q) red[q] = tot[q]; if (errsrc) red[nq] = *errsrc; return; }
-    cg_logic(op, tot, nq, cg, out, tol, maxit);
+    cg_logic(op, tot, nq, cg, out, tol, maxit, 0.0, ah);
 }
 __global__ void k_cg_logic(int op, const double *__restrict__ red, int nq, CgScalars *__restrict__ cg, double *__restrict__ out,
-                           double tol, int maxit, int with_flag)
+                           double tol, int maxit, int with_flag, double *__restrict__ ah = nullptr)
 {
     if (op == FIN_PAP || op == FIN_RR) { if (cg->done) return; }
     double tot[4] = { 0, 0, 0, 0 };
     for (int q = 0; q < nq; ++q) tot[q] = red[q];
-    cg_logic(op, tot, nq, cg, out, tol, maxit, with_flag ? red[nq] : 0.0);
+    cg_logic(op, tot, nq, cg, out, tol, maxit, with_flag ? red[nq] : 0.0, ah);
     if (with_flag == 2) out[nq] = red[nq];
 }
 
@@ -599,7 +600,8 @@
 }
 __device__ __forceinline__ void sto(double *p, unsigned byte_off, double v) { *reinterpret_cast<double *>(reinterpret_cast<char *>(p) + byte_off) = v; }
 
-struct CgFuse { double *p; const double *r; double *xsol; double *pout; };
+enum { XB_NOW = 0, XB_SKIP = 1, XB_APPLY = 2 };
+struct CgFuse { double *p; const double *r; double *xsol; double *pout; int nold; int a0; const double *ah; const double *old[7]; };
 
 struct LineDict { const int *id = nullptr; int pitch = 0; };
 struct LineFp { unsigned long long lo, hi; };
@@ -665,7 +667,7 @@
     if (tC) tC[i] = in ? Cd[e] : 0.0;
 }
 
-template <int K, int NCH, bool VEC, int NB, class Mid = NoMid, bool DPPS = false, bool NT = false, bool DICT = false>
+template <int K, int NCH, bool VEC, int NB, class Mid = NoMid, bool DPPS = false, bool NT = false, bool DICT = false, int XB = XB_NOW>
 __device__ __forceinline__ double schur_x_task(const ModeArgs &ma, const Geom &G, const double *__restrict__ L, const double *__restrict__ DR,
                                                const double *__restrict__ D0, int nx, int ny, long nlines, int lpl_log2, int first,
                                                long task, int lane, bool active, bool fuse, double f_alpha, double f_beta, const CgFuse &fz, Mid mid = Mid(),
@@ -673,6 +675,7 @@
 {
     static_assert(K == 2, "two cells per lane and chunk");
     static_assert(!DICT || (NB == 0 && NT), "line tables: next to the streaming RT0-P0 instantiations only");
+    static_assert(XB == XB_NOW || NB == 0, "batched x_sol update: RT0-P0 only");
     const int LPL = 1 << lpl_log2, LPW = 64 >> lpl_log2;
     const int li = lane & (LPL - 1), sub = lane >> lpl_log2;
     const long line = task * LPW + sub;
@@ -699,12 +702,17 @@
             if (fuse) {
                 const long mo = (ma.x[q] - fz.p) + base + c0;
                 ld2<NT>(fz.r, mo, ok, VEC, rq[q][ch][0], rq[q][ch][1], ok2);
-                ld2<NT>(fz.xsol, mo, ok, VEC, sq[q][ch][0], sq[q][ch][1], ok2);
+                if (XB != XB_SKIP) ld2<NT>(fz.xsol, mo, ok, VEC, sq[q][ch][0], sq[q][ch][1], ok2);
             }
         }
         if (NB > 0) ld2<NT>(ma.D, base + c0, ok, VEC, dq[NB > 0 ? ch : 0][0], dq[NB > 0 ? ch : 0][1], ok2);
     }
     if (mid(f_alpha, f_beta)) return 0.0;
+    double av[7];
+    if (XB == XB_APPLY) {
+#pragma unroll
+        for (int i = 0; i < 7; ++i) av[i] = i < fz.nold ? fz.ah[(fz.a0 + i) & 7] : 0.0;
+    }
 #pragma unroll
     for (int ch = 0; ch < NCH; ++ch) {
         const int c0 = (ch * LPL + li) * K;
@@ -713,14 +721,22 @@
 #pragma unroll
             for (int q = 0; q <= NB; ++q) {
                 const long mo = (ma.x[q] - fz.p) + base + c0;
-                const double s0 = fma(f_alpha, xm[q][ch][0], sq[q][ch][0]), s1 = fma(f_alpha, xm[q][ch][1], sq[q][ch][1]);
+                if (XB == XB_APPLY) {
+                    double o0[7], o1[7];
+#pragma unroll
+                    for (int i = 0; i < 7; ++i) if (i < fz.nold) ld2<NT>(fz.old[i], mo, ok, VEC, o0[i], o1[i], ok2);
+#pragma unroll
+                    for (int i = 0; i < 7; ++i) if (i < fz.nold) { sq[q][ch][0] = fma(av[i], o0[i], sq[q][ch][0]); sq[q][ch][1] = fma(av[i], o1[i], sq[q][ch][1]); }
+                }
+                double s0 = 0.0, s1 = 0.0;
+                if (XB != XB_SKIP) { s0 = fma(f_alpha, xm[q][ch][0], sq[q][ch][0]); s1 = fma(f_alpha, xm[q][ch][1], sq[q][ch][1]); }
                 xm[q][ch][0] = fma(f_beta, xm[q][ch][0], rq[q][ch][0]); xm[q][ch][1] = fma(f_beta, xm[q][ch][1], rq[q][ch][1]);
                 if (VEC) {
-                    if (ok) { *reinterpret_cast<double2 *>(fz.xsol + mo) = make_double2(s0, s1);
+                    if (ok) { if (XB != XB_SKIP) *reinterpret_cast<double2 *>(fz.xsol + mo) = make_double2(s0, s1);
                               *reinterpret_cast<double2 *>(pw + mo) = make_double2(xm[q][ch][0], xm[q][ch][1]); }
                 } else {
-                    if (ok) { fz.xsol[mo] = s0; pw[mo] = xm[q][ch][0]; }
-                    if (ok2) { fz.xsol[mo + 1] = s1; pw[mo + 1] = xm[q][ch][1]; }
+                    if (ok) { if (XB != XB_SKIP) fz.xsol[mo] = s0; pw[mo] = xm[q][ch][0]; }
+                    if (ok2) { if (XB != XB_SKIP) fz.xsol[mo + 1] = s1; pw[mo + 1] = xm[q][ch][1]; }
                 }
             }
         }
@@ -818,7 +834,7 @@
     return dot;
 }
 
-template <int K, int NCH, bool VEC, int NB, bool NT = false, bool DICT = false>
+template <int K, int NCH, bool VEC, int NB, bool NT = false, bool DICT = false, int XB = XB_NOW>
 __global__ __launch_bounds__(256) void k_schur_x(ModeArgs ma0, ModeTab mt, Geom G, const double *__restrict__ L, const double *__restrict__ DR,
                                                  const double *__restrict__ D0, int nx, int ny, long nlines, int lpl_log2,
                                                  int first, int last, double *__restrict__ partials,
@@ -840,7 +856,7 @@
     };
     unsigned bx = blockIdx.x;
     if ((first & 2) && gridDim.x % 8 == 0) bx = (blockIdx.x % 8) * (gridDim.x / 8) + blockIdx.x / 8;
-    const double dot = schur_x_task<K, NCH, VEC, NB, decltype(mid), false, NT, DICT>(ma, G, L, DR, D0, nx, ny, nlines, lpl_log2, first & 1, (long)bx * 4 + (threadIdx.x >> 6),
+    const double dot = schur_x_task<K, NCH, VEC, NB, decltype(mid), false, NT, DICT, XB>(ma, G, L, DR, D0, nx, ny, nlines, lpl_log2, first & 1, (long)bx * 4 + (threadIdx.x >> 6),
                                                                            threadIdx.x & 63, true, fuse, alpha0, beta0, fz, mid, ld);
     if (stopped) return;
     if (last && partials) {
@@ -2060,11 +2076,24 @@
     s = block_sum(s, sred);
     if (threadIdx.x == 0) partials[blockIdx.x] = s;
 }
-__global__ void k_cg_flush(double *__restrict__ x, const double *__restrict__ p, long n, const CgScalars *__restrict__ cg)
-{
-    if (!cg->pend) return;
-    const double alpha = cg->alpha;
-    for (long i = blockIdx.x * 256L + threadIdx.x; i < n; i += gridDim.x * 256L) x[i] = fma(alpha, p[i], x[i]);
+struct FlushRing { int n; int alpha[8]; const double *ah; const double *p[8]; };
+__global__ void k_cg_flush(double *__restrict__ x, const double *__restrict__ p, long n, const CgScalars *__restrict__ cg, FlushRing ring)
+{
+    if (ring.n < 0) {
+        if (!cg->pend) return;
+        const double alpha = cg->alpha;
+        for (long i = blockIdx.x * 256L + threadIdx.x; i < n; i += gridDim.x * 256L) x[i] = fma(alpha, p[i], x[i]);
+        return;
+    }
+    double a[8];
+#pragma unroll
+    for (int j = 0; j < 8; ++j) a[j] = j < ring.n ? ring.ah[ring.alpha[j] & 7] : 0.0;
+    for (long i = blockIdx.x * 256L + threadIdx.x; i < n; i += gridDim.x * 256L) {
+        double v = x[i];
+#pragma unroll
+        for (int j = 0; j < 8; ++j) if (j < ring.n) v = fma(a[j], ring.p[j][i], v);
+        x[i] = v;
+    }
 }
 __global__ __launch_bounds__(256) void k_cg_pupdate(double *__restrict__ p, const double *__restrict__ r, long n,
                                                     const CgScalars *__restrict__ cg)
diff --git a/neutfem_amd/csrc/nf_options.h b/neutfem_amd/csrc/nf_options.h
--- a/neutfem_amd/csrc/nf_options.h
+++ b/neutfem_amd/csrc/nf_options.h
@@ -15,6 +15,7 @@
     long prof_every = 8;
     long cg_batch = 0;
     long nt_loads = 1, nt_min_cells = 8000000;
+    long xsol_batch = -1;
     long cg_fuse = 1;
     long xcd = -1;
     long outer_dev = 1;
@@ -122,9 +123,19 @@
     *n = (int)(sizeof rows / sizeof rows[0]);
     return rows;
 }
+inline const NfOptionRow *nf_option_rows_more(int *n)
+{
+    static const NfOptionRow rows[] = {
+        { "xsol_batch", &NfOptions::xsol_batch, NF_CLAMP, -1, 8, NF_COPY_SOLVE, 0, nullptr, nullptr },
+    };
+    *n = (int)(sizeof rows / sizeof rows[0]);
+    return rows;
+}
 inline const NfOptionRow *nf_option_find(const char *key)
 {
     int n = 0; const NfOptionRow *rows = nf_option_rows(&n);
+    for (int i = 0; i < n; ++i) if (!strcmp(key, rows[i].key)) return rows + i;
+    rows = nf_option_rows_more(&n);
     for (int i = 0; i < n; ++i) if (!strcmp(key, rows[i].key)) return rows + i;
     return nullptr;
 }
@@ -157,12 +168,14 @@
 }
 inline unsigned nf_options_copy(NfOptions &dst, const NfOptions &src, bool same_mesh_kind)
 {
-    int n = 0; const NfOptionRow *rows = nf_option_rows(&n);
     unsigned fx = 0;
-    for (int i = 0; i < n; ++i) {
-        const NfOptionRow &r = rows[i];
-        if (r.copy == NF_COPY_NONE || (r.copy == NF_COPY_PASS && !same_mesh_kind) || dst.*r.field == src.*r.field) continue;
-        dst.*r.field = src.*r.field; fx |= r.effects;
+    for (int part = 0; part < 2; ++part) {
+        int n = 0; const NfOptionRow *rows = part ? nf_option_rows_more(&n) : nf_option_rows(&n);
+        for (int i = 0; i < n; ++i) {
+            const NfOptionRow &r = rows[i];
+            if (r.copy == NF_COPY_NONE || (r.copy == NF_COPY_PASS && !same_mesh_kind) || dst.*r.field == src.*r.field) continue;
+            dst.*r.field = src.*r.field; fx |= r.effects;
+        }
     }
     return fx & (NF_FX_DICT | NF_FX_REGIME);
 }
diff --git a/neutfem_amd/csrc/nf_xsol_ring.h b/neutfem_amd/csrc/nf_xsol_ring.h
--- /dev/null
+++ b/neutfem_amd/csrc/nf_xsol_ring.h
@@ -0,0 +1,23 @@
+#pragma once
+
+constexpr int NF_XSOL_RING_MAX = 8;
+
+struct NfRingUpdate { int slot, alpha; };
+struct NfRingBatch { int n = 0; NfRingUpdate u[NF_XSOL_RING_MAX] = {}; };
+
+inline int nf_ring_alpha(long j) { return (int)(j % NF_XSOL_RING_MAX); }
+inline int nf_ring_read(long k, int M) { return k > 0 ? (int)((k - 1) % M) : 0; }
+inline int nf_ring_write(long k, int M) { return (int)(k % M); }
+inline NfRingBatch nf_ring_range(long lo, long hi, int M)
+{
+    NfRingBatch B;
+    for (long j = lo; j < hi && B.n < NF_XSOL_RING_MAX; ++j) B.u[B.n++] = { (int)(j % M), nf_ring_alpha(j) };
+    return B;
+}
+inline NfRingBatch nf_ring_apply(long k, int M) { return k >= 1 && k % M == 0 ? nf_ring_range(k - M, k, M) : NfRingBatch(); }
+inline NfRingBatch nf_ring_pending(long n, int pend, int M)
+{
+    if (n <= 0) return NfRingBatch();
+    const long lastx = pend ? n - 1 : n;
+    return nf_ring_range(lastx / M * M, n, M);
+}
```

Measured after the change: 5.336 outer-iters/s, median of 6. +4.1%, better.
